# rezashkv/unlearn-ft

Hardware: AMD Instinct MI355X
Metric: bilevel train-step images/sec @512^2 pruned-SD2.1 (higher is better)
Workload: dtype bf16; 1 GPU; BASELINE configs[1] model+batch (MAC-budget-0.55 SD-2.1 student [ratio 0.556, 223.7 GMAC/img] + dense teacher [402.1 GMAC/img], B=8/GPU, 64x64 latents = 512^2 px, losses 1.0 ddpm(min-SNR 5) + 2.0 distill + 0.1 block) under the bilevel cadence of configs[2] (upper concept-suppression step every 10th iteration, second AdamW); global_batch=8, parallelism=dp1, student_params=483766084, weights=random-init, attention_precision=activation dtype, dist_backend=none, rccl_ranks=0, dp_mode=allreduce, teacher_prefetch=True

## Files before the change

include/pdmk.h:

```cpp
#ifndef PDMK_H
#define PDMK_H
#include <stdint.h>
#ifdef __cplusplus
extern "C" {
#endif

#define PDMK_F32 0
#define PDMK_BF16 1

typedef void* pdmk_stream;

int pdmk_version(void);

#define PDMK_A_ROWK 0
#define PDMK_A_CONV 1
#define PDMK_A_COLK 2
#define PDMK_B_ROWK 0
#define PDMK_B_COLK 1
#define PDMK_B_COLK_CONV 2

typedef struct pdmk_gemm_args {
    const void* A;
    const void* B;
    void* C;
    const float* bias;
    const float* rowvec;
    const void* R;
    float* colsum_out;
    int32_t M, N, K;
    int32_t lda, ldb, ldc, ldr;
    int32_t rows_per_b;
    int32_t a_mode, b_mode;
    int32_t conv_b, conv_hi, conv_wi, conv_ci, conv_ho, conv_wo, conv_mode, conv_ld;
    int32_t dtype;
    int32_t out_f32;
    int32_t accumulate;
    int32_t splitk;
    float alpha;
    int32_t ldrv;
    int32_t epilogue;
    int32_t ldc2;
    void* C2;
    int64_t* colstat;
    int32_t cs_ld;
    int32_t cs_col0;
    const float* ln_gamma;
    const float* ln_beta;
    float* ln_stats;
    void* ln_out;
    int32_t ld_ln_out;
    float ln_eps;
} pdmk_gemm_args;
int pdmk_gemm_ln_supported(const pdmk_gemm_args* args);

#define PDMK_EPI_NONE 0
#define PDMK_EPI_GEGLU 1
#define PDMK_EPI_GEGLU_BWD 2

int pdmk_gemm(const pdmk_gemm_args* args, pdmk_stream stream);
int pdmk_conv_up2_supported(int B, int H, int W, int Ci, int Co, int dtype);
int pdmk_groupnorm_apply_colstat(const void* x, void* y, const float* gamma, const float* beta, float* stats, const int64_t* colstat,
                                 int cs_ld, int cs_col0, int B, int HW, int C, int ldx, int ldy, int G, int gs, float eps,
                                 int silu, int dtype, pdmk_stream stream);
int pdmk_up2_pack_weights(const float* w3, void* wp, void* wpt, int Co, int Ci, int dtype, pdmk_stream stream);
int pdmk_up2_combine_wgrad(const float* dwp, float* dw3, int Co, int Ci, pdmk_stream stream);
#define PDMK_COLSTAT_SCALE 1073741824.0
#define PDMK_GEMM_GROUP_MAX 8
int pdmk_gemm_group(const pdmk_gemm_args* args, int n, pdmk_stream stream, int32_t* grouped_out);
int pdmk_gemm_plan(const pdmk_gemm_args* args, pdmk_stream stream, int32_t* splitk_out);
int pdmk_gemm_last_candidate(void);
int pdmk_gemm_candidate_name(int a_mode, int b_mode, int id, char* buf, int n);
int pdmk_splitk_finish(const float* ws, void* C, const float* bias, const float* rowvec, const void* R, int64_t M,
                       int N, int ldc, int ldr, int rows_per_b, int ldrv , int nslab ,
                       int accumulate, int dtype, pdmk_stream stream);
int pdmk_splitk_finish_colstat(const float* ws, void* C, const float* bias, const float* rowvec, const void* R, int64_t M,
                               int N, int ldc, int ldr, int rows_per_b, int ldrv, int nslab, int accumulate, int64_t* colstat,
                               int cs_ld, int cs_col0, int dtype, pdmk_stream stream);
#define PDMK_SLAB_GROUP_MAX 32
typedef struct pdmk_slab_item {
    const float* ws;
    float* dst;
    int64_t n;
    int32_t nslab, pad_;
} pdmk_slab_item;
int pdmk_splitk_finish_group(const pdmk_slab_item* items, int n_items, pdmk_stream stream);
int64_t pdmk_gemm_splitk_workspace_bytes(int64_t M, int N, int splitk);

int pdmk_plan_export(const char* path);
int pdmk_plan_import(const char* path);
int pdmk_plan_size(void);
int pdmk_plan_clear(void);
int pdmk_debug_scratch_violations(void);

int pdmk_groupnorm_fwd(const void* x, void* y, const float* gamma, const float* beta, float* stats, double* ws,
                       int B, int HW, int C, int ldx, int ldy, int G, int gs, float eps, int silu, int dtype,
                       pdmk_stream stream);
int pdmk_groupnorm_bwd(const void* x, const void* dy, void* dx, const float* gamma, const float* beta,
                       const float* stats, float* dgamma, float* dbeta, double* ws, float* part_ws,
                       int64_t part_ws_elems, int B, int HW, int C, int ldx, int lddy, int lddx, int G, int gs,
                       int silu, int accumulate_dx, const void* add, int ldadd, int dtype, pdmk_stream stream);
#define PDMK_PARTIAL_GROUP_MAX 32
typedef struct pdmk_partial_item {
    const float* part;
    float* out0;
    float* out1;
    int32_t nblk, n;
} pdmk_partial_item;
int pdmk_groupnorm_bwd_partial_dims(int B, int HW, int C, int G, int gs, int dtype, int32_t* nblk, int32_t* n);
int pdmk_layernorm_bwd_partial_dims(int M, int C, int32_t* nblk, int32_t* n);
int pdmk_reduce_partials_group(const pdmk_partial_item* items, int n_items, pdmk_stream stream);
int64_t pdmk_groupnorm_workspace_bytes(int B, int G);
int64_t pdmk_groupnorm_bwd_part_workspace_bytes(int G, int gs);

int pdmk_layernorm_fwd(const void* x, void* y, const float* gamma, const float* beta, float* stats, int M, int C,
                       int ldx, int ldy, float eps, int dtype, pdmk_stream stream);
int pdmk_layernorm_bwd(const void* x, const void* dy, void* dx, const float* gamma, const float* stats,
                       float* dgamma, float* dbeta, float* part_ws, int64_t part_ws_elems ,
                       int M, int C, int ldx, int lddy, int lddx, int accumulate_dx, const void* add, int ldadd, int dtype,
                       pdmk_stream stream);
int64_t pdmk_layernorm_bwd_part_workspace_bytes(int M, int C);

int pdmk_attn_fwd(const void* q, const void* k, const void* v, void* o, float* lse, int B, int H, int Nq, int Nk,
                  int64_t q_bs, int q_ld, int64_t k_bs, int k_ld, int64_t v_bs, int v_ld, int64_t o_bs, int o_ld,
                  float scale, int dtype, pdmk_stream stream);
int pdmk_attn_bwd(const void* q, const void* k, const void* v, const void* o, const void* d_o, const float* lse,
                  float* delta, void* dq, void* dk, void* dv, int B, int H, int Nq, int Nk, int64_t q_bs, int q_ld,
                  int64_t k_bs, int k_ld, int64_t v_bs, int v_ld, int64_t o_bs, int o_ld, int64_t dq_bs, int dq_ld,
                  int64_t dk_bs, int dk_ld, int64_t dv_bs, int dv_ld, float scale, float* ws, int64_t ws_elems,
                  int dtype, pdmk_stream stream);
int64_t pdmk_attn_bwd_workspace_bytes(int B, int H, int Nq, int Nk);

int pdmk_geglu_fwd(const void* x, void* y, int M, int F, int ldx, int ldy, int layout, int dtype, pdmk_stream stream);
int pdmk_geglu_bwd(const void* x, const void* dy, void* dx, int M, int F, int ldx, int lddy, int lddx, int layout,
                   int dtype, pdmk_stream stream);
int pdmk_silu_fwd(const void* x, void* y, int64_t n, int dtype, pdmk_stream stream);
int pdmk_quantize_e4m3(const void* x, void* y, int64_t n, int dtype, pdmk_stream stream);
int pdmk_silu_bwd(const void* x, const void* dy, void* dx, int64_t n, int dtype, pdmk_stream stream);
int pdmk_copy2d(const void* src, void* dst, int64_t rows, int cols, int lds, int ldd, int accumulate, int dtype,
                pdmk_stream stream);
int pdmk_cast_permute(const float* src, void* dst, int n0, int n1, int n2, int mode, int dtype, pdmk_stream stream);
int pdmk_colsum(const void* x, float* out, int64_t rows, int N, int ld, int accumulate, int nbatch, int ldo , int dtype, pdmk_stream stream);
int pdmk_pool2x2_sum(const void* src, void* dst, int B, int H, int W, int C, int dtype, pdmk_stream stream);
int pdmk_timestep_embed(const int64_t* t, const float* freqs, void* out, int B, int dim, int dtype,
                        pdmk_stream stream);
int pdmk_add_noise_velocity(const float* x0, const float* noise, const int64_t* t, const float* sqrt_acp,
                            const float* sqrt_1macp, void* noisy_nhwc, float* target_nhwc, int B, int C, int HW,
                            int cpad, int dtype, pdmk_stream stream);
int pdmk_nchw_to_nhwc(const float* src, void* dst, int B, int C, int HW, int cpad, int dtype, pdmk_stream stream);
int pdmk_nhwc_to_nchw(const void* src, float* dst, int B, int C, int HW, int ld, int dtype, pdmk_stream stream);

int pdmk_mse_fwd(const void* a, int a_dtype, const void* b, int b_dtype, const float* w, double* out, int slot,
                 int B, int64_t rows_per_b, int cols, int lda, int ldb, double scale, pdmk_stream stream);
int pdmk_mse_bwd(const void* a, int a_dtype, const void* b, int b_dtype, const float* w, void* da, int B,
                 int64_t rows_per_b, int cols, int lda, int ldb, int ldda, float gscale, int accumulate,
                 pdmk_stream stream);
int pdmk_mse_fwd_bwd(const void* a, int a_dtype, const void* b, int b_dtype, const float* w, double* out, int slot,
                     void* da, int B, int64_t rows_per_b, int cols, int lda, int ldb, int ldda, double scale,
                     float gscale, int accumulate, pdmk_stream stream);
int pdmk_zero(void* p, int64_t nbytes, pdmk_stream stream);
int pdmk_axpby(const void* x, void* y, float alpha, float beta, int64_t n, int dtype, pdmk_stream stream);

int pdmk_adamw(float* p, float* g, float* m, float* v, int64_t n, const float* lr, float beta1, float beta2,
               float eps, float weight_decay, const float* bias_corr , float grad_scale,
               int zero_grad, void* w_bf16 , pdmk_stream stream);
int pdmk_transpose_tiles(const void* src, void* dst, const int32_t* table, int ntiles, int dtype, pdmk_stream stream);
int pdmk_skinny_gemm(const void* x, int x_dtype, const void* w, void* y, const float* bias, int M, int N, int K,
                     int ldx, int ldw, int ldy, int dtype, int out_f32, int accumulate, pdmk_stream stream);
int pdmk_skinny_wgrad(const void* dy, int dy_dtype, const void* x, float* dw, float* dbias, int M, int N, int K,
                      int lddy, int ldx, int lddw, int dtype, pdmk_stream stream);
int pdmk_sumsq(const float* x, int64_t n, double* out, int slot, pdmk_stream stream);

int pdmk_softmax_rows(const float* s, void* p, int64_t rows, int cols, int64_t lds, int64_t ldp, int dtype,
                      pdmk_stream stream);
int pdmk_latent_sample(const void* moments, int ld, const float* eps, float* latents, int B, int C, int HW, float scale,
                       int dtype, pdmk_stream stream);

int pdmk_embed_tokens(const int64_t* ids, const void* tok, const void* pos, void* out, int64_t ntok, int T, int D,
                      int vocab, int ldt, int ldp, int ldo, int dtype, pdmk_stream stream);
int pdmk_attn_fwd_causal(const void* q, const void* k, const void* v, void* o, float* lse, int B, int H, int N,
                         int64_t q_bs, int q_ld, int64_t k_bs, int k_ld, int64_t v_bs, int v_ld, int64_t o_bs, int o_ld,
                         float scale, int dtype, pdmk_stream stream);
int pdmk_gelu_fwd(const void* x, void* y, int64_t n, int dtype, pdmk_stream stream);

typedef struct {
    int64_t offset;
    int64_t h, w;
    int64_t rh, rw;
    int64_t top, left;
    int64_t flip;
} pdmk_image_desc;
int pdmk_image_prep(const uint8_t* src, int64_t src_bytes, const pdmk_image_desc* desc, const pdmk_image_desc* desc_dev,
                    int B, int R, float* out, pdmk_stream stream);
int pdmk_image_prep_ex(const uint8_t* src, int64_t src_bytes, const pdmk_image_desc* desc, const pdmk_image_desc* desc_dev,
                       int B, int R, int filter, const float* mean, const float* stdv, float* out, pdmk_stream stream);

int pdmk_patch_im2col(const float* x, void* out, int B, int S, int p, int ldo, int dtype, pdmk_stream stream);
int pdmk_vit_tokens(const void* patches, int ldp, const void* cls, const void* pos, int ldpos, void* out, int ldo, int B,
                    int G2, int E, int dtype, pdmk_stream stream);
int pdmk_quick_gelu_fwd(const void* x, void* y, int64_t n, int dtype, pdmk_stream stream);
int pdmk_gather_rows(const void* x, int ldx, const int64_t* ids, int T, void* out, int ldo, int B, int D, int dtype,
                     pdmk_stream stream);
int pdmk_clip_score_head(const float* a, int lda, const float* b, int ldb, float* an, float* bn, double* acc, int B, int D,
                         pdmk_stream stream);

typedef struct {
    int64_t t;
    int32_t mode;
    int32_t nterms;
    int32_t wslot;
    int32_t rslot[3];
    float coef[4];
    float v_x, v_v;
    float eps_scale, x_scale;
    int32_t vpred;
    int32_t pad_;
} pdmk_plms_row;

int pdmk_plms_step(const void* pred, int ld, float g_u, float g_t, int cfg, float* sample, float* cur, float* ets,
                   const pdmk_plms_row* table, int nsteps, int32_t* state, int64_t* t_out, void* x_next, int cpad,
                   int B, int C, int HW, int dtype, pdmk_stream stream);

int pdmk_image_to_u8(const float* src, uint8_t* dst, int B, int C, int HW, pdmk_stream stream);
// ... 30 lines not shown
```

unlearn-ft_amd/csrc/gemm.hip:

```cpp
#include <cstdio>
#include <cstdlib>
#include <cstring>
#include <map>
#include <mutex>
#include <vector>

#include "common.h"
#include <algorithm>

namespace {

#define PDMK_GEMM_NBUF 2
#ifndef PDMK_GEMM_PF2
#define PDMK_GEMM_PF2 0
#endif
constexpr int BM = 128, BN = 128;
template <typename T, int KCHUNKS, int NW> struct TileCfg {
    static constexpr int NTHREADS = 64 * NW;
    static constexpr int IM = 8 / NW * 2;
    static constexpr int TPR = NTHREADS / 128;
    static constexpr int NLD = KCHUNKS / TPR;
    static constexpr int ROW_BYTES = KCHUNKS == 8 ? 144 : 96;
    static constexpr int OPERAND_BYTES = 128 * ROW_BYTES;
    static constexpr int CH = Mma<T>::CH;
// ... 276 lines not shown
                for (int h = 0; h < 2; ++h) {
                    const int n = n0 + h * 64 + lane;
                    if (n < g.N) {
                        float v = stage[lrow * SROW + h * 64 + lane];
                        if (first) {
                            if (g.bias) v += g.bias[n];
                            if (g.rowvec) v += g.rowvec[(long)(m / g.rows_per_b) * (g.ldrv ? g.ldrv : g.N) + n];
                            if (Rp) v += to_f32(Rp[(long)m * g.ldr + n]);
                        }
                        unsafeAtomicAdd(Cf + (long)m * g.ldc + n, v);
                    }
                }
            }
        } else {
            constexpr int TPS = NTHREADS / 64, SEG = 128 / TPS;
            const int lrow = tid / TPS, seg = (tid % TPS) * SEG;
            const int m = m0 + pass * 64 + lrow;
            if (m < g.M) {
                const float* rv = g.rowvec ? g.rowvec + (long)(m / g.rows_per_b) * (g.ldrv ? g.ldrv : g.N) : nullptr;
#pragma unroll
                for (int c8 = 0; c8 < SEG / 8; ++c8) {
                    const int n = n0 + seg + c8 * 8;
                    if (n >= g.N) break;
                    float v[8];
                    const f32x4 lo = *reinterpret_cast<const f32x4*>(stage + lrow * SROW + seg + c8 * 8);
                    const f32x4 hi = *reinterpret_cast<const f32x4*>(stage + lrow * SROW + seg + c8 * 8 + 4);
#pragma unroll
                    for (int r = 0; r < 4; ++r) { v[r] = lo[r]; v[4 + r] = hi[r]; }
                    const long off = (long)m * g.ldc + n;
                    if (vec8) {
                        if (g.bias) {
                            const float4 b0 = *reinterpret_cast<const float4*>(g.bias + n), b1 = *reinterpret_cast<const float4*>(g.bias + n + 4);
                            v[0] += b0.x; v[1] += b0.y; v[2] += b0.z; v[3] += b0.w; v[4] += b1.x; v[5] += b1.y; v[6] += b1.z; v[7] += b1.w;
                        }
                        if (rv) {
                            const float4 b0 = *reinterpret_cast<const float4*>(rv + n), b1 = *reinterpret_cast<const float4*>(rv + n + 4);
                            v[0] += b0.x; v[1] += b0.y; v[2] += b0.z; v[3] += b0.w; v[4] += b1.x; v[5] += b1.y; v[6] += b1.z; v[7] += b1.w;
                        }
                        if (Rp) {
                            if (sizeof(T) == 2) {
                                const bf16x8 rr = *reinterpret_cast<const bf16x8*>(Rp + (long)m * g.ldr + n);
#pragma unroll
                                for (int r = 0; r < 8; ++r) v[r] += (float)rr[r];
                            } else {
                                const float* rp = reinterpret_cast<const float*>(Rp) + (long)m * g.ldr + n;
                                const float4 b0 = *reinterpret_cast<const float4*>(rp), b1 = *reinterpret_cast<const float4*>(rp + 4);
                                v[0] += b0.x; v[1] += b0.y; v[2] += b0.z; v[3] += b0.w; v[4] += b1.x; v[5] += b1.y; v[6] += b1.z; v[7] += b1.w;
                            }
                        }
                        if (f32out) {
                            float4 o0 = make_float4(v[0], v[1], v[2], v[3]), o1 = make_float4(v[4], v[5], v[6], v[7]);
                            if (acc1) {
                                const float4 c0 = *reinterpret_cast<const float4*>(Cf + off), c1 = *reinterpret_cast<const float4*>(Cf + off + 4);
                                o0.x += c0.x; o0.y += c0.y; o0.z += c0.z; o0.w += c0.w; o1.x += c1.x; o1.y += c1.y; o1.z += c1.z; o1.w += c1.w;
                            }
                            *reinterpret_cast<float4*>(Cf + off) = o0;
                            *reinterpret_cast<float4*>(Cf + off + 4) = o1;
                        } else {
                            if (acc1) {
                                const bf16x8 c = *reinterpret_cast<const bf16x8*>(Ct + off);
#pragma unroll
                                for (int r = 0; r < 8; ++r) v[r] += (float)c[r];
                            }
                            bf16x8 o;
#pragma unroll
                            for (int r = 0; r < 8; ++r) o[r] = (bf16)v[r];
                            st_stream(reinterpret_cast<bf16x8*>(Ct + off), o);
                        }
                    } else {
                        const int nv = min(8, g.N - n);
                        for (int r = 0; r < nv; ++r) {
                            float x = v[r];
                            if (g.bias) x += g.bias[n + r];
                            if (rv) x += rv[n + r];
                            if (Rp) x += to_f32(Rp[(long)m * g.ldr + n + r]);
                            if (f32out) Cf[off + r] = x + (acc1 ? Cf[off + r] : 0.f);
                            else Ct[off + r] = from_f32<T>(x + (acc1 ? to_f32(Ct[off + r]) : 0.f));
                        }
                    }
                }
            }
        }
    }
}

inline int ilog2_exact(int v) {
    if (v <= 0 || (v & (v - 1))) return -1;
    int l = 0;
    while ((1 << l) < v) ++l;
    return l;
}

template <typename T> int launch(const pdmk_gemm_args& g, hipStream_t st) {
    const int mt = (g.M + BM - 1) / BM, nt = (g.N + BN - 1) / BN;
    dim3 grid(mt * nt, g.splitk > 1 ? g.splitk : 1);
    int lg_wo = -1, lg_howo = -1;
    if (g.b_mode == PDMK_B_COLK_CONV) {
        lg_wo = ilog2_exact(g.conv_wo);
        lg_howo = ilog2_exact(g.conv_ho * g.conv_wo);
        if (lg_wo < 0 || lg_howo < 0) lg_wo = lg_howo = -1;
    }
    const long esz = sizeof(T);
    const long conv_bytes = (((long)g.conv_b * g.conv_hi * g.conv_wi - 1) * g.conv_ld + g.conv_ci) * esz;
    const long a_bytes = g.a_mode == PDMK_A_ROWK ? ((long)(g.M - 1) * g.lda + g.K) * esz
                       : g.a_mode == PDMK_A_CONV ? conv_bytes : ((long)(g.K - 1) * g.lda + g.M) * esz;
    const long b_bytes = g.b_mode == PDMK_B_ROWK ? ((long)(g.N - 1) * g.ldb + g.K) * esz
                       : g.b_mode == PDMK_B_COLK ? ((long)(g.K - 1) * g.ldb + g.N) * esz : conv_bytes;
    if (a_bytes >= (1L << 31) || b_bytes >= (1L << 31)) return -1;
    const bool many = (long)grid.x * grid.y > 512;
    const bool deep4 = false;
#define PDMK_GO(AM, BMD, CM)                                                                                        \
    do {                                                                                                            \
        if (deep4)                                                                                                  \
            hipLaunchKernelGGL((igemm_kernel<T, AM, BMD, CM, 4, 4>), grid, dim3(256), 0, st, g, lg_wo, lg_howo,     \
                               (unsigned)a_bytes, (unsigned)b_bytes);                                               \
        else if (many)                                                                                              \
            hipLaunchKernelGGL((igemm_kernel<T, AM, BMD, CM, 4, 8>), grid, dim3(512), 0, st, g, lg_wo, lg_howo,     \
                               (unsigned)a_bytes, (unsigned)b_bytes);                                               \
        else                                                                                                        \
            hipLaunchKernelGGL((igemm_kernel<T, AM, BMD, CM, 8, 8>), grid, dim3(512), 0, st, g, lg_wo, lg_howo,     \
                               (unsigned)a_bytes, (unsigned)b_bytes);                                               \
    } while (0)
    if (g.a_mode == PDMK_A_ROWK && g.b_mode == PDMK_B_ROWK) PDMK_GO(PDMK_A_ROWK, PDMK_B_ROWK, 0);
    else if (g.a_mode == PDMK_A_CONV && g.b_mode == PDMK_B_ROWK) {
        switch (g.conv_mode) {
            case 0: PDMK_GO(PDMK_A_CONV, PDMK_B_ROWK, 0); break;
            case 1: PDMK_GO(PDMK_A_CONV, PDMK_B_ROWK, 1); break;
            case 2: PDMK_GO(PDMK_A_CONV, PDMK_B_ROWK, 2); break;
            case 3: PDMK_GO(PDMK_A_CONV, PDMK_B_ROWK, 3); break;
            default: PDMK_GO(PDMK_A_CONV, PDMK_B_ROWK, 4); break;
        }
    } else if (g.a_mode == PDMK_A_COLK && g.b_mode == PDMK_B_COLK) PDMK_GO(PDMK_A_COLK, PDMK_B_COLK, 0);
    else if (g.a_mode == PDMK_A_COLK && g.b_mode == PDMK_B_COLK_CONV) {
        switch (g.conv_mode) {
            case 0: PDMK_GO(PDMK_A_COLK, PDMK_B_COLK_CONV, 0); break;
            case 1: PDMK_GO(PDMK_A_COLK, PDMK_B_COLK_CONV, 1); break;
            case 2: PDMK_GO(PDMK_A_COLK, PDMK_B_COLK_CONV, 2); break;
            default: return -2;
        }
    } else return -2;
#undef PDMK_GO
    PDMK_CHECK_LAUNCH();
    return 0;
}

}

int pdmk_gemm_dma_launch(const pdmk_gemm_args& g, hipStream_t st, long a_bytes, long b_bytes);
int pdmk_gemm_ring_launch(const pdmk_gemm_args& g, hipStream_t st, long a_bytes, long b_bytes, int id);
int pdmk_gemm_ring_num_configs();
int pdmk_gemm_ring_pick(const pdmk_gemm_args& g);
int pdmk_wgrad_ring_launch(const pdmk_gemm_args& g, hipStream_t st, long a_bytes, long b_bytes, int id);
int pdmk_wgrad_ring_num_configs();

static int env_int(const char* name, int def, int* cache) {
    static int dynamic = -1;
    if (dynamic < 0) dynamic = getenv("PDMK_ENV_DYNAMIC") ? 1 : 0;
    if (*cache == INT32_MIN || dynamic) {
        const char* e = getenv(name);
        *cache = e ? atoi(e) : def;
    }
    return *cache;
}
static int dma_mode() { static int c = INT32_MIN; return env_int("PDMK_GEMM_DMA", 1, &c); }
static int ring_mode() { static int c = INT32_MIN; return env_int("PDMK_GEMM_RING", 1, &c); }
static int tune_mode() { static int c = INT32_MIN; return env_int("PDMK_GEMM_TUNE", 1, &c); }
static int forced_cfg() { static int c = INT32_MIN; return env_int("PDMK_RING_CFG", -1, &c); }
static int forced_wcfg() { static int c = INT32_MIN; return env_int("PDMK_WGRAD_CFG", -1, &c); }

namespace {

struct PlanKey {
    int v[10];
    bool operator<(const PlanKey& o) const { return memcmp(v, o.v, sizeof v) < 0; }
};
std::mutex g_plan_mu;
std::map<PlanKey, int> g_plan_cfg;
std::map<PlanKey, int> g_plan_sk;
thread_local int g_last_candidate = -1;
bool g_plan_file_loaded = false;

void plan_file_load() {
    if (g_plan_file_loaded) return;
    g_plan_file_loaded = true;
    const char* path = getenv("PDMK_PLAN_CACHE");
    if (!path) return;
    FILE* f = fopen(path, "r");
    if (!f) return;
    int ver = 0;
    if (fscanf(f, " pdmk-plan %d", &ver) != 1 || ver != pdmk_version()) {
        fclose(f);
        return;
    }
    char kind;
    PlanKey k;
    int val;
    while (fscanf(f, " %c %d %d %d %d %d %d %d %d %d %d %d", &kind, &k.v[0], &k.v[1], &k.v[2], &k.v[3], &k.v[4], &k.v[5],
                  &k.v[6], &k.v[7], &k.v[8], &k.v[9], &val) == 12) {
        if (kind == 'c') g_plan_cfg[k] = val;
        else if (kind == 's') g_plan_sk[k] = val;
    }
    fclose(f);
}
void plan_file_append(char kind, const PlanKey& k, int val) {
    const char* path = getenv("PDMK_PLAN_CACHE");
    if (!path) return;
    FILE* probe = fopen(path, "r");
    int ver = 0;
    const bool fresh = !probe || fscanf(probe, " pdmk-plan %d", &ver) != 1 || ver != pdmk_version();
    if (probe) fclose(probe);
    FILE* f = fopen(path, fresh ? "w" : "a");
    if (!f) return;
    if (fresh) fprintf(f, "pdmk-plan %d\n", pdmk_version());
    fprintf(f, "%c %d %d %d %d %d %d %d %d %d %d %d\n", kind, k.v[0], k.v[1], k.v[2], k.v[3], k.v[4], k.v[5], k.v[6], k.v[7],
            k.v[8], k.v[9], val);
    fclose(f);
}
void* g_scratch = nullptr;
size_t g_scratch_bytes = 0;

PlanKey make_key(const pdmk_gemm_args& g, int sk) {
    PlanKey k;
    const bool cv = g.a_mode == PDMK_A_CONV || g.b_mode == PDMK_B_COLK_CONV;
    const int slabw = (g.a_mode == PDMK_A_COLK && g.accumulate == 2) ? 1000 : 0;
    const int v[10] = {g.M, g.N, g.K, g.a_mode, g.b_mode, (cv ? g.conv_mode : 100 * g.epilogue) + slabw, cv ? g.conv_hi : 0,
                       cv ? g.conv_wi : 0, cv ? g.conv_ci : 0, sk};
    memcpy(k.v, v, sizeof v);
    return k;
}

bool ring_eligible(const pdmk_gemm_args& g) {
    return g.dtype == PDMK_BF16 && g.b_mode == PDMK_B_ROWK && g.a_mode != PDMK_A_COLK;
}

bool wgrad_eligible(const pdmk_gemm_args& g) {
    return g.dtype == PDMK_BF16 && g.a_mode == PDMK_A_COLK && g.b_mode != PDMK_B_ROWK && g.out_f32 &&
           (g.b_mode == PDMK_B_COLK || g.conv_mode <= 2 || (g.conv_mode >= 5 && g.conv_mode <= 8));
}

bool operand_bytes(const pdmk_gemm_args& g, long* ab, long* bb) {
    const long in_px = (long)g.conv_b * g.conv_hi * g.conv_wi * ((g.a_mode == PDMK_A_CONV && g.conv_mode >= 9) ? 4 : 1);
    const long conv_bytes = ((in_px - 1) * g.conv_ld + g.conv_ci) * 2;
    const long krows = (g.a_mode == PDMK_A_COLK && g.b_mode == PDMK_B_COLK_CONV && g.conv_mode >= 5) ? 4L * g.K : (long)g.K;
    *ab = g.a_mode == PDMK_A_ROWK ? ((long)(g.M - 1) * g.lda + g.K) * 2
        : g.a_mode == PDMK_A_CONV ? conv_bytes : ((krows - 1) * g.lda + g.M) * 2;
    *bb = g.b_mode == PDMK_B_ROWK ? ((long)(g.N - 1) * g.ldb + g.K) * 2
        : g.b_mode == PDMK_B_COLK ? ((long)(g.K - 1) * g.ldb + g.N) * 2 : conv_bytes;
    return *ab < (1L << 31) && *bb < (1L << 31);
}

int launch_legacy(const pdmk_gemm_args& g, hipStream_t st) {
    if (g.colstat) return -2;
    if ((g.a_mode == PDMK_A_CONV || g.b_mode == PDMK_B_COLK_CONV) && g.conv_mode >= 5) return -2;
    const long nblocks = (long)((g.M + 127) / 128) * ((g.N + 127) / 128) * (g.splitk > 1 ? g.splitk : 1);
    long ab, bb;
    if (dma_mode() && (nblocks >= 384 || dma_mode() == 2) && ring_eligible(g) && (g.K % 32) == 0 && operand_bytes(g, &ab, &bb)) {
        const int rc = pdmk_gemm_dma_launch(g, st, ab, bb);
        if (rc <= 0) return rc;
    }
    return g.dtype == PDMK_BF16 ? launch<bf16>(g, st) : launch<float>(g, st);
}

int launch_candidate(const pdmk_gemm_args& g, hipStream_t st, int id) {
    if (id <= 0) return launch_legacy(g, st);
    long ab, bb;
    if (!operand_bytes(g, &ab, &bb)) return 1;
    if (g.a_mode == PDMK_A_COLK) return pdmk_wgrad_ring_launch(g, st, ab, bb, id - 1);
    return pdmk_gemm_ring_launch(g, st, ab, bb, id - 1);
}

static int debug_scratch();
long out_rows(const pdmk_gemm_args& g) {
    const bool phase_fwd = g.a_mode == PDMK_A_CONV && g.conv_mode >= 5 && g.conv_mode <= 8;
    if (phase_fwd && debug_scratch() == 2 && 3L * g.M * g.N * 4 + 4096 <= (1L << 20)) return (long)g.M;
    return phase_fwd ? 4L * g.M : (long)g.M;
}

bool can_tune(hipStream_t st) {
    if (!tune_mode() || !ring_mode()) return false;
    hipStreamCaptureStatus cs = hipStreamCaptureStatusNone;
    if (hipStreamIsCapturing(st, &cs) != hipSuccess) { (void)hipGetLastError(); return false; }
    return cs == hipStreamCaptureStatusNone;
}

constexpr size_t kCanaryBytes = 1 << 20;
size_t g_scratch_req = 0;
int g_scratch_violations = 0;
static int debug_scratch() { static int c = INT32_MIN; return env_int("PDMK_DEBUG_SCRATCH", 0, &c); }
static_assert(kCanaryBytes == (1 << 20), "out_rows() sizes its deliberate overrun against the band");

bool ensure_scratch(size_t bytes) {
    if (debug_scratch()) {
        if (g_scratch) (void)hipFree(g_scratch);
        g_scratch = nullptr;
        g_scratch_bytes = 0;
        bytes = (bytes + 255) & ~(size_t)255;
        if (hipMalloc(&g_scratch, bytes + kCanaryBytes) != hipSuccess) { (void)hipGetLastError(); return false; }
        if (hipMemset(reinterpret_cast<char*>(g_scratch) + bytes, 0xA5, kCanaryBytes) != hipSuccess) { (void)hipGetLastError(); return false; }
        (void)hipDeviceSynchronize();
        g_scratch_bytes = bytes + kCanaryBytes;
        g_scratch_req = bytes;
        return true;
    }
    if (bytes <= g_scratch_bytes) return true;
    if (g_scratch) (void)hipFree(g_scratch);
    g_scratch = nullptr;
// ... 102 lines not shown
    if (s > 64) s = 64;
    return s < 1 ? 1 : s;
}

int heuristic_sk(const pdmk_gemm_args& g) {
    if (g.N & 3) return 1;
    const bool conv0 = g.a_mode == PDMK_A_CONV && g.conv_mode == 0;
    const int bm = conv0 ? (g.M >= 8192 ? 256 : 128) : (g.M >= 8192 ? 128 : 64);
    const int bn = conv0 ? 160 : 128;
    const long tiles = (long)((g.M + bm - 1) / bm) * ((g.N + bn - 1) / bn);
    const int nk = (g.K + 63) / 64;
    if (tiles >= 160 || nk < 30) return 1;
    long s = (256 + tiles - 1) / tiles;
    if (s > nk / 8) s = nk / 8;
    if (conv0 && s > (g.conv_ci + 63) / 64) s = (g.conv_ci + 63) / 64;
    return s < 1 ? 1 : (s > 16 ? 16 : (int)s);
}

}

static int validate_args(const pdmk_gemm_args& g) {
    if (!g.A || !g.B || !g.C) return -1;
    if (g.M <= 0 || g.N <= 0 || g.K <= 0) return -1;
    const int ch = g.dtype == PDMK_BF16 ? 8 : 4;
    const int g4 = 4 * ch;
    if (g.dtype != PDMK_BF16 && g.dtype != PDMK_F32) return -2;
    if (g.a_mode != PDMK_A_COLK && (g.K % g4)) return -1;
    if (((uintptr_t)g.A | (uintptr_t)g.B) & 15) return -1;
    if (g.a_mode == PDMK_A_ROWK && (g.lda % ch)) return -1;
    if (g.a_mode == PDMK_A_COLK && ((g.lda % ch) || (g.M % g4))) return -1;
    if (g.b_mode == PDMK_B_ROWK && (g.ldb % ch)) return -1;
    if (g.b_mode == PDMK_B_COLK && ((g.ldb % ch) || (g.N % g4))) return -1;
    if (g.a_mode == PDMK_A_CONV || g.b_mode == PDMK_B_COLK_CONV) {
        if (g.conv_ci <= 0 || (g.conv_ci % g4) || (g.conv_ld % ch) || g.conv_mode < 0 || g.conv_mode > 13) return -1;
        if (g.conv_mode >= 5) {
            if (g.dtype != PDMK_BF16 || g.conv_ho != g.conv_hi || g.conv_wo != g.conv_wi) return -2;
            if (g.b_mode == PDMK_B_COLK_CONV && g.conv_mode > 8) return -1;
        }
        if (g.conv_mode == 4 && (g.b_mode == PDMK_B_COLK_CONV || (g.conv_hi & 1) || (g.conv_wi & 1))) return -1;
        if (g.conv_b <= 0 || g.conv_hi <= 0 || g.conv_wi <= 0 || g.conv_ho <= 0 || g.conv_wo <= 0) return -1;
        const long px = (long)g.conv_b * g.conv_ho * g.conv_wo;
        if (px >= (1L << 30) || (long)g.conv_b * g.conv_hi * g.conv_wi >= (1L << 30)) return -1;
        const int ntaps = g.conv_mode == 13 ? 16 : (g.conv_mode >= 5 ? 4 : 9);
        if (g.a_mode == PDMK_A_CONV && (g.M != px || g.K != ntaps * g.conv_ci)) return -1;
        if (g.b_mode == PDMK_B_COLK_CONV && (g.K != px || g.N != ntaps * g.conv_ci)) return -1;
        if (g.conv_mode >= 5 && (long)g.conv_b * g.conv_hi * g.conv_wi * 4 >= (1L << 30)) return -1;
        const bool half = g.conv_mode == 1 || g.conv_mode == 4, twice = g.conv_mode == 2 || g.conv_mode == 3;
        const int eh = half ? (g.conv_hi + 1) / 2 : (twice ? 2 * g.conv_hi : g.conv_hi);
        const int ew = half ? (g.conv_wi + 1) / 2 : (twice ? 2 * g.conv_wi : g.conv_wi);
        if (g.conv_ho != eh || g.conv_wo != ew) return -1;
    }
    if (g.splitk > 1 && !(g.out_f32 || g.dtype == PDMK_F32)) return -1;
    if (g.accumulate == 2 && (g.splitk <= 1 || !(g.out_f32 || g.dtype == PDMK_F32) || g.bias || g.rowvec || g.R)) return -1;
    if (g.accumulate < 0 || g.accumulate > 2) return -1;
    if (g.rowvec && g.rows_per_b <= 0) return -1;
    if (g.epilogue != PDMK_EPI_NONE) {
        if (g.epilogue != PDMK_EPI_GEGLU && g.epilogue != PDMK_EPI_GEGLU_BWD) return -2;
        if (g.dtype != PDMK_BF16 || g.a_mode != PDMK_A_ROWK || g.b_mode != PDMK_B_ROWK || g.out_f32) return -2;
        if (g.epilogue == PDMK_EPI_GEGLU) {
            if ((g.N % 16) || (g.ldc % 8) || (g.C2 && (g.ldc2 % 8)) || g.splitk > 1 || g.accumulate || g.R || g.rowvec ||
                g.alpha != 1.0f || (g.K % 8))
                return -1;
        } else {
            if ((g.N % 8) || (g.ldc % 8) || !g.C2 || (g.ldc2 % 8) || g.splitk > 1 || g.accumulate || g.R || g.rowvec || g.bias ||
                g.alpha != 1.0f || (g.K % 8) || (((uintptr_t)g.C2 | (uintptr_t)g.C) & 15))
                return -1;
        }
        if (!ring_mode()) return -2;
    }
    if (g.colstat) {
        if (g.dtype != PDMK_BF16 || g.a_mode == PDMK_A_COLK || g.b_mode != PDMK_B_ROWK || g.out_f32 || g.epilogue) return -2;
        if (g.rows_per_b <= 0 || (g.rows_per_b % 64) || (g.M % 64) || (g.N % 8) || (g.ldc % 8) || (g.R && (g.ldr % 8)) ||
            g.splitk > 1 || g.accumulate == 2 || g.cs_col0 < 0 || g.cs_ld < g.cs_col0 + g.N || (g.K % 8))
            return -1;
        if (g.a_mode == PDMK_A_CONV && g.conv_mode >= 9) return -1;
        if (!ring_mode()) return -2;
    }
    return 0;
}

int pdmk_gemm_rowblock_launch(const pdmk_gemm_args& g, hipStream_t st, long a_bytes, long b_bytes, int id, bool dry);
int pdmk_gemm_rowblock_num_configs();
static int ln_candidate(const pdmk_gemm_args& g, long* ab, long* bb) {
    if (g.dtype != PDMK_BF16 || g.a_mode != PDMK_A_ROWK || g.b_mode != PDMK_B_ROWK || g.splitk > 1 || g.colstat || g.out_f32 ||
        !ring_mode() || !operand_bytes(g, ab, bb))
        return -1;
    for (int id = 0; id < pdmk_gemm_rowblock_num_configs(); ++id)
        if (pdmk_gemm_rowblock_launch(g, nullptr, *ab, *bb, id, true) == 0) return id;
    return -1;
}
extern "C" int pdmk_gemm_ln_supported(const pdmk_gemm_args* a) {
    if (!a || !a->ln_gamma || validate_args(*a)) return 0;
    long ab, bb;
    return ln_candidate(*a, &ab, &bb) >= 0 ? 1 : 0;
}

extern "C" int pdmk_gemm(const pdmk_gemm_args* a, pdmk_stream stream) {
    if (!a) return -1;
    const pdmk_gemm_args& g = *a;
    if (const int vrc = validate_args(g)) return vrc;
    hipStream_t st = reinterpret_cast<hipStream_t>(stream);
    g_last_candidate = 0;
    if (g.ln_gamma) {
        long ab, bb;
        const int id = ln_candidate(g, &ab, &bb);
        if (id < 0) return -2;
        const int rc = pdmk_gemm_rowblock_launch(g, st, ab, bb, id, false);
        g_last_candidate = 1 + pdmk_gemm_ring_num_configs() - pdmk_gemm_rowblock_num_configs() + id;
        return rc == 1 ? -2 : rc;
    }
    if (!(ring_eligible(g) && (g.K % 8) == 0) && !wgrad_eligible(g)) return launch_legacy(g, st);
    if ((g.a_mode == PDMK_A_COLK ? forced_wcfg() >= 0 : forced_cfg() >= 0) && !(g.epilogue && forced_cfg() == 0)) {
        const int rc = launch_candidate(g, st, g.a_mode == PDMK_A_COLK ? forced_wcfg() : forced_cfg());
        g_last_candidate = rc == 1 ? 0 : (g.a_mode == PDMK_A_COLK ? forced_wcfg() : forced_cfg());
        if (g.epilogue && rc == 1) return -2;
        const bool phase = (g.a_mode == PDMK_A_CONV || g.b_mode == PDMK_B_COLK_CONV) && g.conv_mode >= 5;
        if (!((phase || g.colstat) && rc == 1)) return rc == 1 ? launch_legacy(g, st) : rc;
    }
    const int sk = g.splitk > 1 ? g.splitk : 1;
    int id;
    {
        std::lock_guard<std::mutex> lk(g_plan_mu);
        plan_file_load();
        const PlanKey key = make_key(g, sk);
        auto it = g_plan_cfg.find(key);
        if (it != g_plan_cfg.end()) id = it->second;
        else if (can_tune(st)) {
            float t;
            id = tune_cfg(g, st, sk, &t);
            if (id < 0) id = heuristic_cfg(g);
            g_plan_cfg[key] = id;
            plan_file_append('c', key, id);
        } else id = heuristic_cfg(g);
    }
    if ((g.epilogue || g.colstat) && id <= 0) id = 1 + pdmk_gemm_ring_pick(g);
    int rc = launch_candidate(g, st, id);
    if (g.colstat && rc == 1) {
        id = 1 + pdmk_gemm_ring_pick(g);
        rc = launch_candidate(g, st, id);
    }
    if (g.epilogue && rc == 1) return -2;
    g_last_candidate = rc == 1 ? 0 : id;
    return rc == 1 ? launch_legacy(g, st) : rc;
}

int pdmk_gemm_ring_group_launch(const pdmk_gemm_args* gs, int n, hipStream_t st, const long* a_bytes, const long* b_bytes, int id);
int pdmk_wgrad_ring_group_launch(const pdmk_gemm_args* gs, int n, hipStream_t st, const long* a_bytes, const long* b_bytes, int id);
static int group_mode() { static int c = INT32_MIN; return env_int("PDMK_GEMM_GROUP", 1, &c); }
static int forced_group() { static int c = INT32_MIN; return env_int("PDMK_GROUP_CFG", -1, &c); }

namespace {

std::map<std::vector<int>, int> g_group_plan;

int member_plan(const pdmk_gemm_args& g, hipStream_t st) {
    const int sk = g.splitk > 1 ? g.splitk : 1;
    std::lock_guard<std::mutex> lk(g_plan_mu);
    plan_file_load();
    const PlanKey key = make_key(g, sk);
    auto it = g_plan_cfg.find(key);
    if (it != g_plan_cfg.end()) return it->second;
    if (!can_tune(st)) return heuristic_cfg(g);
    float t;
    int id = tune_cfg(g, st, sk, &t);
    if (id < 0) id = heuristic_cfg(g);
    g_plan_cfg[key] = id;
    plan_file_append('c', key, id);
    return id;
}

int group_launch(const pdmk_gemm_args* a, int n, hipStream_t st, int id) {
    long ab[PDMK_GEMM_GROUP_MAX], bb[PDMK_GEMM_GROUP_MAX];
    for (int i = 0; i < n; ++i)
        if (!operand_bytes(a[i], &ab[i], &bb[i])) return 1;
    if (id <= 0) return 1;
    if (a[0].a_mode == PDMK_A_COLK) return pdmk_wgrad_ring_group_launch(a, n, st, ab, bb, id - 1);
    return pdmk_gemm_ring_group_launch(a, n, st, ab, bb, id - 1);
}

template <typename F> float time_us(F fn, hipStream_t st, hipEvent_t e0, hipEvent_t e1, int reps = 3) {
    if (fn() != 0) { (void)hipGetLastError(); return 1e30f; }
    float best = 1e30f;
    for (int round = 0; round < 2; ++round) {
        (void)hipEventRecord(e0, st);
        for (int r = 0; r < reps; ++r)
            if (fn() != 0) { (void)hipGetLastError(); return 1e30f; }
        (void)hipEventRecord(e1, st);
        if (hipEventSynchronize(e1) != hipSuccess) { (void)hipGetLastError(); return 1e30f; }
        float ms = 0.f;
        (void)hipEventElapsedTime(&ms, e0, e1);
        if (ms < best) best = ms;
    }
    return best * 1000.f / reps;
}

int tune_group(const pdmk_gemm_args* a, int n, const int* ids, hipStream_t st) {
    pdmk_gemm_args t[PDMK_GEMM_GROUP_MAX];
    size_t off[PDMK_GEMM_GROUP_MAX + 1];
    off[0] = 0;
    for (int i = 0; i < n; ++i) {
        const size_t out = (size_t)out_rows(a[i]) * (size_t)a[i].N * 4;
        const size_t slabs = (a[i].accumulate == 2 && a[i].splitk > 1) ? (size_t)a[i].splitk : 1;
        off[i + 1] = off[i] + ((out * slabs + (size_t)a[i].M * 4 + 1023) & ~(size_t)1023);
    }
    {
        std::lock_guard<std::mutex> lk(g_plan_mu);
        if (!ensure_scratch(off[n] + 256)) return -1;
    }
    (void)hipDeviceSynchronize();
    for (int i = 0; i < n; ++i) {
        t[i] = a[i];
        char* base = reinterpret_cast<char*>(g_scratch) + off[i];
        t[i].C = base;
        t[i].ldc = a[i].N;
        t[i].colstat = nullptr;
        if (t[i].epilogue == PDMK_EPI_GEGLU_BWD) t[i].ldc = 2 * a[i].N;
        else t[i].C2 = nullptr;
        if (t[i].accumulate == 1) t[i].accumulate = 0;
        if (t[i].epilogue == PDMK_EPI_GEGLU) t[i].ldc = a[i].N / 2;
        if (t[i].colsum_out)
            t[i].colsum_out = reinterpret_cast<float*>(base + (off[i + 1] - off[i]) - (((size_t)a[i].M * 4 + 15) & ~(size_t)15));
    }
    hipEvent_t e0, e1;
    if (hipEventCreate(&e0) != hipSuccess || hipEventCreate(&e1) != hipSuccess) { (void)hipGetLastError(); return -1; }
    const float t_sep = time_us([&]() -> int {
        for (int i = 0; i < n; ++i) {
            int rc = launch_candidate(t[i], st, ids[i]);
            if (rc == 1) rc = launch_legacy(t[i], st);
            if (rc) return rc;
        }
        return 0;
    }, st, e0, e1);
    int best = -1;
    float bt = t_sep * 0.98f;
    int cands[PDMK_GEMM_GROUP_MAX + 12], nc = 0;
    for (int i = 0; i < n; ++i) cands[nc++] = ids[i];
    cands[nc++] = heuristic_cfg(a[0]);
    if (a[0].a_mode == PDMK_A_CONV)
        for (int h = 0; h < 4; ++h) cands[nc++] = 1 + 12 + h;
    if (a[0].a_mode == PDMK_A_COLK && a[0].b_mode == PDMK_B_COLK)
        for (int w = 0; w < 5; ++w) cands[nc++] = 1 + w;
    for (int i = 0; i < nc; ++i) {
        bool seen = cands[i] <= 0;
        for (int j = 0; j < i; ++j) seen = seen || cands[j] == cands[i];
        if (seen) continue;
        const float tg = time_us([&]() -> int { return group_launch(t, n, st, cands[i]); }, st, e0, e1);
        if (tg < bt) { bt = tg; best = cands[i]; }
    }
    (void)hipEventDestroy(e0);
    (void)hipEventDestroy(e1);
    if (getenv("PDMK_TUNE_LOG")) {
        fprintf(stderr, "[pdmk group] n=%d", n);
        for (int i = 0; i < n; ++i) fprintf(stderr, " (%d,%d,%d|a%d sk%d id%d)", a[i].M, a[i].N, a[i].K, a[i].a_mode, a[i].splitk, ids[i]);
        fprintf(stderr, " separate %.1f us -> %s %d (%.1f us)\n", t_sep, best > 0 ? "grouped cand" : "separate", best, best > 0 ? bt : t_sep);
    }
    {
        std::lock_guard<std::mutex> lk(g_plan_mu);
        if (!scratch_check()) return -1;
    }
    return best;
}

}

extern "C" int pdmk_gemm_group(const pdmk_gemm_args* a, int n, pdmk_stream stream, int32_t* grouped_out) {
    if (grouped_out) *grouped_out = 0;
    if (!a || n < 1 || n > PDMK_GEMM_GROUP_MAX) return -1;
    bool any_ln = false;
    for (int i = 0; i < n; ++i) {
        if (const int vrc = validate_args(a[i])) return vrc;
        any_ln = any_ln || a[i].ln_gamma;
    }
    hipStream_t st = reinterpret_cast<hipStream_t>(stream);
    auto separate = [&]() -> int {
        for (int i = 0; i < n; ++i)
            if (const int rc = pdmk_gemm(&a[i], stream)) return rc;
        return 0;
    };
    if (n > 1 && forced_group() >= 1 && !any_ln) {
        const int rc = group_launch(a, n, st, forced_group());
        if (rc == 0) {
            g_last_candidate = forced_group();
            if (grouped_out) *grouped_out = n;
            return 0;
        }
        return rc == 1 ? separate() : rc;
    }
    if (n == 1 || any_ln || !group_mode() || !ring_mode() || forced_cfg() >= 0 || forced_wcfg() >= 0) return separate();
    bool fw = true, wg = true;
    for (int i = 0; i < n; ++i) {
        fw = fw && ring_eligible(a[i]) && (a[i].K % 8) == 0 && (a[i].a_mode == a[0].a_mode);
        wg = wg && wgrad_eligible(a[i]) && (a[i].b_mode == a[0].b_mode);
    }
    if (!fw && !wg) return separate();
    int ids[PDMK_GEMM_GROUP_MAX];
    std::vector<int> key;
    for (int i = 0; i < n; ++i) {
        ids[i] = member_plan(a[i], st);
        if ((a[i].epilogue || a[i].colstat) && ids[i] <= 0) ids[i] = 1 + pdmk_gemm_ring_pick(a[i]);
        const PlanKey k = make_key(a[i], a[i].splitk > 1 ? a[i].splitk : 1);
        key.insert(key.end(), k.v, k.v + 10);
        key.push_back(a[i].accumulate);
    }
    int id = -2;
    {
        std::lock_guard<std::mutex> lk(g_plan_mu);
        auto it = g_group_plan.find(key);
        if (it != g_group_plan.end()) id = it->second;
    }
    if (id == -2) {
        if (can_tune(st)) {
            id = tune_group(a, n, ids, st);
            std::lock_guard<std::mutex> lk(g_plan_mu);
            g_group_plan[key] = id;
        } else {
            id = ids[0];
            for (int i = 1; i < n; ++i)
                if (ids[i] != ids[0]) id = -1;
        }
    }
    if (id > 0) {
        const int rc = group_launch(a, n, st, id);
        if (rc == 0) {
            g_last_candidate = id;
            if (grouped_out) *grouped_out = n;
            return 0;
        }
        if (rc != 1) return rc;
    }
    return separate();
}

extern "C" int pdmk_gemm_last_candidate(void) { return g_last_candidate; }
int pdmk_gemm_ring_name(int id, int conv, char* buf, int n);
int pdmk_wgrad_ring_name(int id, int conv, char* buf, int n);
extern "C" int pdmk_gemm_candidate_name(int a_mode, int b_mode, int id, char* buf, int n) {
    if (!buf || n <= 0) return -1;
    if (id <= 0) {
        snprintf(buf, n, "igemm_kernel / pdmk_dma::igemm_dma_kernel (K-step-32)");
        return 0;
    }
    if (a_mode == PDMK_A_COLK) return pdmk_wgrad_ring_name(id - 1, b_mode == PDMK_B_COLK_CONV, buf, n);
    return pdmk_gemm_ring_name(id - 1, a_mode == PDMK_A_CONV, buf, n);
}

extern "C" int pdmk_gemm_plan(const pdmk_gemm_args* a, pdmk_stream stream, int32_t* splitk_out) {
    if (!a || !splitk_out) return -1;
    const pdmk_gemm_args& g = *a;
    hipStream_t st = reinterpret_cast<hipStream_t>(stream);
    *splitk_out = 1;
    if (g.M <= 0 || g.N <= 0 || g.K <= 0) return -1;
    if ((g.N & 3) || g.epilogue) return 0;
    const bool wg = wgrad_eligible(g);
    if (g.a_mode == PDMK_A_COLK && !wg) {
        *splitk_out = heuristic_wgrad_sk(g);
        return 0;
    }
    if (!wg && (!ring_eligible(g) || (g.K % 8) || forced_cfg() >= 0)) {
        *splitk_out = heuristic_sk(g);
        return 0;
    }
    std::lock_guard<std::mutex> lk(g_plan_mu);
    plan_file_load();
    const PlanKey key0 = make_key(g, 0);
    auto it = g_plan_sk.find(key0);
    if (it != g_plan_sk.end()) { *splitk_out = it->second; return 0; }
    if (!can_tune(st) || !a->A || !a->B) { *splitk_out = wg ? heuristic_wgrad_sk(g) : heuristic_sk(g); return 0; }
    const int tiles = ((g.M + 127) / 128) * ((g.N + 127) / 128);
    const int nk = (g.K + 63) / 64;
    const int cands[12] = {1, 2, 3, 4, 6, 8, 12, 16, 24, 32, 48, 64};
    int best_sk = 1;
    float bt = 1e30f;
    for (int c = 0; c < 12; ++c) {
        const int sk = cands[c];
        if (wg) {
            if (sk > 1 && (nk / sk < 4 || (long)tiles * sk > 1280)) continue;
            if ((long)tiles * sk * 4 < 128 && sk < 64 && nk / (2 * sk) >= 4) continue;
        } else if (sk > 16 || (sk > 1 && (tiles > 200 || nk < 10 || nk / sk < 3 || (long)tiles * sk > 768))) continue;
        float t = 1e30f;
        const int id = tune_cfg(g, st, sk, &t);
        if (id < 0) continue;
        g_plan_cfg[make_key(g, sk)] = id;
        plan_file_append('c', make_key(g, sk), id);
        static const float margin = getenv("PDMK_SPLIT_MARGIN") ? 1.0f - 0.01f * (float)atof(getenv("PDMK_SPLIT_MARGIN")) : 0.97f;
        if (t < bt * (sk > 1 ? margin : 1.0f)) { bt = t; best_sk = sk; }
    }
    g_plan_sk[key0] = best_sk;
    plan_file_append('s', key0, best_sk);
    *splitk_out = best_sk;
    return 0;
}

extern "C" int pdmk_plan_size(void) {
    std::lock_guard<std::mutex> lk(g_plan_mu);
    return (int)(g_plan_cfg.size() + g_plan_sk.size());
}
extern "C" int pdmk_plan_export(const char* path) {
    if (!path) return -1;
    std::lock_guard<std::mutex> lk(g_plan_mu);
    FILE* f = fopen(path, "w");
    if (!f) return -1;
    fprintf(f, "pdmk-plan %d\n", pdmk_version());
    for (int pass = 0; pass < 2; ++pass)
        for (const auto& kv : (pass ? g_plan_sk : g_plan_cfg)) {
            const PlanKey& k = kv.first;
            fprintf(f, "%c %d %d %d %d %d %d %d %d %d %d %d\n", pass ? 's' : 'c', k.v[0], k.v[1], k.v[2], k.v[3], k.v[4], k.v[5],
                    k.v[6], k.v[7], k.v[8], k.v[9], kv.second);
        }
    return fclose(f) == 0 ? 0 : -1;
}
extern "C" int pdmk_plan_import(const char* path) {
    if (!path) return -1;
    std::lock_guard<std::mutex> lk(g_plan_mu);
    FILE* f = fopen(path, "r");
    if (!f) return -1;
    int ver = 0;
    if (fscanf(f, " pdmk-plan %d", &ver) != 1 || ver != pdmk_version()) {
        fclose(f);
        return -2;
    }
    char kind;
    PlanKey k;
    int val, n = 0;
    while (fscanf(f, " %c %d %d %d %d %d %d %d %d %d %d %d", &kind, &k.v[0], &k.v[1], &k.v[2], &k.v[3], &k.v[4], &k.v[5],
                  &k.v[6], &k.v[7], &k.v[8], &k.v[9], &val) == 12) {
        if (kind == 'c') g_plan_cfg[k] = val;
        else if (kind == 's') g_plan_sk[k] = val;
        ++n;
    }
    fclose(f);
    return n;
}
extern "C" int pdmk_plan_clear(void) {
    std::lock_guard<std::mutex> lk(g_plan_mu);
    g_plan_cfg.clear();
    g_plan_sk.clear();
    g_group_plan.clear();
    if (g_scratch) (void)hipFree(g_scratch);
    g_scratch = nullptr;
    g_scratch_bytes = 0;
    return 0;
}

extern "C" int pdmk_debug_scratch_violations(void) {
    std::lock_guard<std::mutex> lk(g_plan_mu);
    return g_scratch_violations;
}

extern "C" int pdmk_version(void) { return 121; }
```

unlearn-ft_amd/csrc/gemm_ring.hip:

```cpp
#include "common.h"

#include <stdio.h>
#include <stdlib.h>

#ifndef PDMK_WGRAD_XCD
#define PDMK_WGRAD_XCD 1
#endif
#ifndef PDMK_HALO_PAIRS
#define PDMK_HALO_PAIRS 1
#endif
#ifndef PDMK_RING_SPLIT_ISSUE
#define PDMK_RING_SPLIT_ISSUE 0
#endif
#ifndef PDMK_HALO_SPLIT_ISSUE
#define PDMK_HALO_SPLIT_ISSUE 1
#endif

#ifndef PDMK_PRIO
#define PDMK_PRIO 0
#endif

namespace pdmk_ring {

constexpr int BK = 64, NT = 512;
constexpr unsigned OOB = 0x80000000u;
typedef __attribute__((address_space(3))) void lds_void;

struct ConvGeom {
    int hi, wi, ci, ho, wo, ld, mode;
};

struct LC {
    unsigned bx, by, gx, gy;
};
__device__ __forceinline__ LC lc_plain() { return LC{blockIdx.x, blockIdx.y, gridDim.x, gridDim.y}; }
__device__ __forceinline__ LC lc_split_xcd() {
    const unsigned gx = gridDim.x, gy = gridDim.y;
    if (gy == 1) return LC{blockIdx.x, 0u, gx, 1u};
    const unsigned t = (unsigned)xcd_remap((int)(blockIdx.y * gx + blockIdx.x), (int)(gx * gy));
    const unsigned z = t / gx;
    return LC{t - z * gx, z, gx, gy};
}
__device__ __forceinline__ bool lc_group(const pdmk_gemm_group_dev& gg, int& pi, LC& lc) {
    const unsigned b = blockIdx.x;
    pi = 0;
#pragma unroll
    for (int i = 1; i < PDMK_GEMM_GROUP_MAX; ++i)
        if (i < gg.n && b >= (unsigned)gg.start[i]) pi = i;
    const unsigned local = b - (unsigned)gg.start[pi];
    const unsigned gx = (unsigned)gg.gx[pi], gy = (unsigned)gg.gy[pi];
    if (local >= gx * gy) return false;
    const unsigned t = gy > 1 ? (unsigned)xcd_remap((int)local, (int)(gx * gy)) : local;
    const unsigned z = t / gx;
    lc = LC{t - z * gx, z, gx, gy};
    return true;
}

__device__ __forceinline__ int conv_src_pixel(const ConvGeom& g, int b, int oy, int ox, int tap) {
    if (g.mode >= 5) {
        const int ph = g.mode - 5, vy = oy + (tap >> 1) - 1 + (ph >> 1), vx = ox + (tap & 1) - 1 + (ph & 1);
        const bool ok = (unsigned)vy < (unsigned)g.hi && (unsigned)vx < (unsigned)g.wi && tap < 4;
        return ok ? (b * g.hi + vy) * g.wi + vx : -1;
    }
    const int ky = (tap * 11) >> 5;
    const int kx = tap - 3 * ky;
    const bool s2 = g.mode == 1 || g.mode == 4, up = g.mode == 2 || g.mode == 3;
    const int pad = g.mode == 4 ? 0 : 1;
    const int vy = (s2 ? 2 * oy : oy) + ky - pad, vx = (s2 ? 2 * ox : ox) + kx - pad;
    const int hv = up ? 2 * g.hi : g.hi, wv = up ? 2 * g.wi : g.wi;
    bool ok = (unsigned)vy < (unsigned)hv && (unsigned)vx < (unsigned)wv && tap < 9;
    if (g.mode == 3) ok = ok && (((vy | vx) & 1) == 0);
    const int iy = up ? (vy >> 1) : vy, ix = up ? (vx >> 1) : vx;
    return ok ? (b * g.hi + iy) * g.wi + ix : -1;
}

__device__ __forceinline__ void wait_vmcnt_dyn(int n) { pdmk_wait_vmcnt(n); }
__device__ __forceinline__ void prio_static(int wave) {
    if (PDMK_PRIO == 1 && wave >= 4) __builtin_amdgcn_s_setprio(1);
}
#define PDMK_PRIO_UP() do { if (PDMK_PRIO == 2) __builtin_amdgcn_s_setprio(1); } while (0)
#define PDMK_PRIO_DOWN() do { if (PDMK_PRIO == 2) __builtin_amdgcn_s_setprio(0); } while (0)

template <int BM, int NJ, int LDS_BYTES, bool TILE2D = false, bool OUTMAP = false>
__device__ __forceinline__ void ring_epilogue(const pdmk_gemm_args& g, const LC wgc, f32x4 (&acc)[BM / 64][NJ], unsigned char* smem,
                                              int m0, int n0, int tw = 0, int img_w = 0) {
    auto row_of = [&](int l) { return TILE2D ? m0 + (l / tw) * img_w + (l % tw) : m0 + l; };
    auto out_row = [&](int m) -> long {
        if (!OUTMAP) return (long)m;
        const int hw = g.conv_hi * g.conv_wi, b = m / hw, rem = m - b * hw, y = rem / g.conv_wi, x = rem - y * g.conv_wi;
        const int ph = g.conv_mode - 5;
        return ((long)(b * 2 * g.conv_hi + 2 * y + (ph >> 1)) * (2 * g.conv_wi) + 2 * x + (ph & 1));
    };
    constexpr int BN = 32 * NJ, IM = BM / 64;
    const int tid = threadIdx.x, lane = tid & 63, wave = __builtin_amdgcn_readfirstlane(tid >> 6);
    const int wm = wave >> 1, wn = wave & 1;
    const bool first = wgc.by == 0;
    const bool slab = g.accumulate == 2;
    const bool atomic = wgc.gy > 1 && !slab;
    const bool acc1 = g.accumulate == 1;
    const bool f32out = g.out_f32 != 0;
    const bool vec8 = ((g.N & 7) == 0) && ((g.ldc & 7) == 0) && (g.R == nullptr || (g.ldr & 7) == 0);
    constexpr int SROW = BN + 4;
    constexpr int C8 = BN / 8;
    constexpr int ITEMS = (64 * C8 + NT - 1) / NT;
    constexpr int RS = NT / C8, CS_STRIDE = RS * C8, ITEMS_CS = (64 + RS - 1) / RS;
    constexpr bool CS_OK = RS * 2 * BN * 4 <= LDS_BYTES;
    static_assert(ITEMS_CS >= ITEMS && (CS_OK || NJ < 2), "statistics epilogue of the forward tile shapes");
    float* stage = reinterpret_cast<float*>(smem);
    static_assert(64 * SROW * 4 <= LDS_BYTES, "staging image must fit the ring");
    float* Cf = reinterpret_cast<float*>(g.C) + (slab ? (long)wgc.by * g.M * g.ldc : 0L);
    bf16* Ct = reinterpret_cast<bf16*>(g.C);
    const bf16* Rp = reinterpret_cast<const bf16*>(g.R);
    float cs1[8] = {0.f, 0.f, 0.f, 0.f, 0.f, 0.f, 0.f, 0.f}, cs2[8] = {0.f, 0.f, 0.f, 0.f, 0.f, 0.f, 0.f, 0.f};
#pragma unroll
    for (int pass = 0; pass < BM / 64; ++pass) {
        __syncthreads();
        if ((wm * 16 * IM) / 64 == pass) {
            const int lrb = (wm * 16 * IM) % 64;
#pragma unroll
            for (int i = 0; i < IM; ++i)
#pragma unroll
                for (int j = 0; j < NJ; ++j) {
                    f32x4 v = acc[i][j];
#pragma unroll
                    for (int r = 0; r < 4; ++r) v[r] *= g.alpha;
                    *reinterpret_cast<f32x4*>(stage + (lrb + i * 16 + (lane & 15)) * SROW + wn * (16 * NJ) + j * 16 + (lane >> 4) * 4) = v;
                }
        }
        if (atomic) {
            __syncthreads();
            for (int rr = 0; rr < 8; ++rr) {
                const int lr2 = wave * 8 + rr, m = row_of(pass * 64 + lr2);
                if (m >= g.M) break;
#pragma unroll
                for (int h = 0; h < (BN + 63) / 64; ++h) {
                    const int cl = h * 64 + lane, n = n0 + cl;
                    if (cl < BN && n < g.N) {
                        float v = stage[lr2 * SROW + cl];
                        if (first) {
                            if (g.bias) v += g.bias[n];
                            if (g.rowvec) v += g.rowvec[(long)(m / g.rows_per_b) * (g.ldrv ? g.ldrv : g.N) + n];
                            if (Rp) v += (float)Rp[(long)m * g.ldr + n];
                        }
                        unsafeAtomicAdd(Cf + (long)m * g.ldc + n, v);
                    }
                }
            }
        } else if (vec8 && g.epilogue == PDMK_EPI_GEGLU) {
            constexpr int C16 = BN / 16;
            constexpr int ITEMS2 = (64 * C16 + NT - 1) / NT;
            bf16* C2 = reinterpret_cast<bf16*>(g.C2);
            __syncthreads();
#pragma unroll
            for (int it = 0; it < ITEMS2; ++it) {
                const int item = tid + it * NT;
                const int lr2 = item / C16, p = item - lr2 * C16;
// ... 656 lines not shown
    const int per = (nk_total + wgc.gy - 1) / wgc.gy;
    const int kt0 = wgc.by * per;
    const int kt1 = min(nk_total, kt0 + per);
    if (kt0 >= kt1 && g.accumulate != 2) return;

    const auto rsrcA = __builtin_amdgcn_make_buffer_rsrc(const_cast<void*>(g.A), (short)0, (int)a_bytes, 0x00020000);
    const auto rsrcB = __builtin_amdgcn_make_buffer_rsrc(const_cast<void*>(g.B), (short)0, (int)b_bytes, 0x00020000);
    const ConvGeom cg{g.conv_hi, g.conv_wi, g.conv_ci, g.conv_ho, g.conv_wo, g.conv_ld, g.conv_mode};

    auto lane_row = [&](int rbytes) { return rbytes == 256 ? (lane >> 4) : (lane >> 3); };
    auto lane_lc = [&](int rbytes) {
        if (rbytes == 256) return (lane & 15) ^ (((lane >> 4) | (((wave >> 1) & 1) << 2)) << 1);
        return (lane & 7) ^ (((((lane >> 3) >> 1) & 1) | ((wave & 1) << 1)) << 1);
    };
    const int a_row = lane_row(RA), b_rowl = lane_row(RB);
    const int acol = m0 + lane_lc(RA) * 8, bcol = n0 + lane_lc(RB) * 8;
    const bool a_ok = acol < g.M, b_ok = bcol < g.N;
    int b_tap = 0, b_ci = 0;
    if (CONV) {
        b_tap = bcol / cg.ci;
        b_ci = bcol - b_tap * cg.ci;
    }

    auto issue = [&](int kt, int slot) {
        unsigned char* sa = smem + slot * SLOT;
#pragma unroll
        for (int i = 0; i < PA; ++i) {
            const int piece = i * 8 + wave;
            const int kr = kt * BK + piece * (1024 / RA) + a_row;
            unsigned krs = (unsigned)kr;
            if (CONV && cg.mode >= 5 && kr < g.K) {
                const int hw = cg.ho * cg.wo, b = kr / hw, rem = kr - b * hw, oy = rem / cg.wo, ox = rem - oy * cg.wo;
                const int ph = cg.mode - 5;
                krs = (unsigned)((b * 2 * cg.ho + 2 * oy + (ph >> 1)) * (2 * cg.wo) + 2 * ox + (ph & 1));
            }
            const unsigned va = (kr < g.K && a_ok) ? (krs * (unsigned)g.lda + (unsigned)acol) * 2u : OOB;
            __builtin_amdgcn_raw_ptr_buffer_load_lds(rsrcA, (lds_void*)(sa + piece * 1024), 16, (int)va, 0, 0, 0);
        }
#pragma unroll
        for (int i = 0; i < PB; ++i) {
            const int piece = i * 8 + wave;
            const int kr = kt * BK + piece * (1024 / RB) + b_rowl;
            const bool kok = kr < g.K;
            unsigned vb = OOB;
            if (CONV) {
                if (kok && b_ok) {
                    int b, oy, ox;
                    if (lg_wo >= 0) {
                        b = kr >> lg_howo;
                        const int rem = kr & ((1 << lg_howo) - 1);
                        oy = rem >> lg_wo;
                        ox = rem & ((1 << lg_wo) - 1);
                    } else {
                        const int hw = cg.ho * cg.wo;
                        b = kr / hw;
                        const int rem = kr - b * hw;
                        oy = rem / cg.wo;
                        ox = rem - oy * cg.wo;
                    }
                    const int px = conv_src_pixel(cg, b, oy, ox, b_tap);
                    if (px >= 0) vb = ((unsigned)px * (unsigned)cg.ld + (unsigned)b_ci) * 2u;
                }
            } else if (kok && b_ok) {
                vb = ((unsigned)kr * (unsigned)g.ldb + (unsigned)bcol) * 2u;
            }
            __builtin_amdgcn_raw_ptr_buffer_load_lds(rsrcB, (lds_void*)(sa + A_BYTES + piece * 1024), 16, (int)vb, 0, 0, 0);
        }
    };

    f32x4 acc[IM][NJ], acs[IM];
#pragma unroll
    for (int i = 0; i < IM; ++i) {
        acs[i] = f32x4{0.f, 0.f, 0.f, 0.f};
#pragma unroll
        for (int j = 0; j < NJ; ++j) acc[i][j] = f32x4{0.f, 0.f, 0.f, 0.f};
    }
    const bool do_colsum = g.colsum_out != nullptr && n0 == 0 && wn == 0;
    bf16x8 ones;
#pragma unroll
    for (int e = 0; e < 8; ++e) ones[e] = (bf16)1.0f;

    const int tg = lane >> 4, tq = (lane & 15) >> 2, tp = lane & 3;
    const int f256 = (tq | ((tg & 1) << 2)) << 1, f128 = (((tq >> 1) & 1) | ((tg & 1) << 1)) << 1;
    typedef __attribute__((address_space(3))) s16x4 lds_s16x4;
    auto tr_frag = [&](const unsigned char* base, int rbytes, int kk, int col0) -> bf16x8 {
        const unsigned ch = (unsigned)(((col0 >> 3) ^ (rbytes == 256 ? f256 : f128)) | (tp >> 1));
        const unsigned char* a0 = base + (unsigned)(kk + 8 * tg + tq) * (unsigned)rbytes + ch * 16u + (unsigned)(tp & 1) * 8u;
        s16x4 lo = __builtin_amdgcn_ds_read_tr16_b64_v4i16((lds_s16x4*)(a0));
        s16x4 hi = __builtin_amdgcn_ds_read_tr16_b64_v4i16((lds_s16x4*)(a0 + 4 * rbytes));
        s16x8 v = __builtin_shufflevector(lo, hi, 0, 1, 2, 3, 4, 5, 6, 7);
        return __builtin_bit_cast(bf16x8, v);
    };

#pragma unroll
    for (int s = 0; s < STAGES - 1; ++s)
        if (kt0 + s < kt1) issue(kt0 + s, s);

    int slot = 0;
    prio_static(wave);
    for (int kt = kt0; kt < kt1; ++kt) {
        if (STAGES == 2) asm volatile("s_waitcnt vmcnt(0)" ::: "memory");
        else if (kt + STAGES - 1 <= kt1) asm volatile("s_waitcnt vmcnt(%0)" ::"n"((STAGES - 2) * (PA + PB)) : "memory");
        else wait_vmcnt_dyn(min(STAGES - 2, kt1 - 1 - kt) * (PA + PB));
        __builtin_amdgcn_s_barrier();
        if (kt + STAGES - 1 < kt1) issue(kt + STAGES - 1, slot == 0 ? STAGES - 1 : slot - 1);
        const unsigned char* sa = smem + slot * SLOT;
        const unsigned char* sb = sa + A_BYTES;
#pragma unroll
        for (int kk = 0; kk < BK; kk += 32) {
            bf16x8 af[IM], bf[NJ];
#pragma unroll
            for (int i = 0; i < IM; ++i) af[i] = tr_frag(sa, RA, kk, wm * (16 * IM) + i * 16);
#pragma unroll
            for (int j = 0; j < NJ; ++j) bf[j] = tr_frag(sb, RB, kk, wn * (16 * NJ) + j * 16);
            PDMK_PRIO_UP();
#pragma unroll
            for (int i = 0; i < IM; ++i)
#pragma unroll
                for (int j = 0; j < NJ; ++j) acc[i][j] = MM::mma(bf[j], af[i], acc[i][j]);
            PDMK_PRIO_DOWN();
            if (do_colsum) {
#pragma unroll
                for (int i = 0; i < IM; ++i) acs[i] = MM::mma(ones, af[i], acs[i]);
            }
        }
        slot = slot + 1 == STAGES ? 0 : slot + 1;
    }
    if (PDMK_PRIO == 1) __builtin_amdgcn_s_setprio(0);
    if (do_colsum && (lane >> 4) == 0) {
#pragma unroll
        for (int i = 0; i < IM; ++i) {
            const int m = m0 + wm * (16 * IM) + i * 16 + (lane & 15);
            if (m < g.M) unsafeAtomicAdd(g.colsum_out + m, acs[i][0]);
        }
    }
    ring_epilogue<BM, NJ, STAGES * SLOT>(g, wgc, acc, smem, m0, n0);
}

template <bool CONV, int BM, int NJ, int STAGES, int OCC>
__global__ __launch_bounds__(NT, OCC) void wgrad_ring_kernel(pdmk_gemm_args g, int lg_wo, int lg_howo, unsigned a_bytes,
                                                             unsigned b_bytes) {
    __shared__ __attribute__((aligned(1024))) unsigned char smem[wgrad_smem_bytes(BM, NJ, STAGES)];
    wgrad_ring_body<CONV, BM, NJ, STAGES, OCC>(g, lg_wo, lg_howo, a_bytes, b_bytes, PDMK_WGRAD_XCD ? lc_split_xcd() : lc_plain(), smem);
}
template <bool CONV, int BM, int NJ, int STAGES, int OCC>
__global__ __launch_bounds__(NT, OCC) void wgrad_ring_group_kernel(pdmk_gemm_group_dev gg) {
    __shared__ __attribute__((aligned(1024))) unsigned char smem[wgrad_smem_bytes(BM, NJ, STAGES)];
    int pi;
    LC wgc;
    if (!lc_group(gg, pi, wgc)) return;
    wgrad_ring_body<CONV, BM, NJ, STAGES, OCC>(gg.p[pi], gg.aux0[pi], gg.aux1[pi], gg.a_bytes[pi], gg.b_bytes[pi], wgc, smem);
}

struct Config {
    int bm, nj, stages, occ;
};
static const Config kConfigs[] = {
    {256, 4, 3, 2}, {256, 5, 3, 2}, {128, 4, 4, 2}, {128, 5, 4, 2}, {64, 4, 6, 2}, {64, 5, 5, 2},
    {128, 4, 2, 4}, {64, 4, 3, 4},  {64, 5, 2, 4},  {128, 6, 3, 2}, {64, 6, 4, 2},  {128, 5, 2, 4},
    {64, 2, 4, 4},  {128, 2, 3, 4}, {64, 3, 4, 4},
};
constexpr int kNumConfigs = sizeof(kConfigs) / sizeof(kConfigs[0]);
constexpr int kNumBase = 12;

static int halo_tile_w(const pdmk_gemm_args& g, int h, int splitk) {
    const bool phase = g.conv_mode >= 5 && g.conv_mode <= 13;
    if (g.a_mode != PDMK_A_CONV || !(g.conv_mode == 0 || phase) || g.conv_ho != g.conv_hi || g.conv_wo != g.conv_wi) return 0;
    if (phase && (h < 2 || !PDMK_HALO_PAIRS || g.R || (splitk > 1))) return 0;
    if ((g.conv_ci % 8) || g.conv_wi < 4) return 0;
    if (phase ? ((g.ldb % 8) || g.ldb < (g.conv_mode == 13 ? 16 : 4) * g.conv_ci) : g.ldb != 9 * g.conv_ci) return 0;
    if ((splitk > 1 ? splitk : 1) > (g.conv_ci + 63) / 64) return 0;
    const int bm = h < 2 ? 256 : 128, pmax = h < 2 ? 400 : 264;
    const int H = g.conv_hi, W = g.conv_wi, HW = H * W;
    if (HW < bm) return (bm % HW) == 0 && (bm / HW) * (H + 2) * (W + 2) <= pmax ? W : 0;
    if (HW % bm) return 0;
    static const int pref = getenv("PDMK_HALO_TW") ? atoi(getenv("PDMK_HALO_TW")) : 0;
    if (pref > 0 && pref < W && (W % pref) == 0 && (bm % pref) == 0 && (H % (bm / pref)) == 0 &&
        (bm / pref + 2) * (pref + 2) <= pmax)
        return pref;
    if ((bm % W) == 0 && (bm / W + 2) * (W + 2) <= pmax) return W;
    for (int tw = 128; tw >= 8; tw >>= 1) {
        if (tw >= W || (W % tw) || (bm % tw)) continue;
        const int rows = bm / tw;
        if ((H % rows) == 0 && (rows + 2) * (tw + 2) <= pmax) return tw;
    }
    return 0;
}
static bool halo_ok(const pdmk_gemm_args& g, int h, int splitk) { return halo_tile_w(g, h, splitk) > 0; }

static int pick_config(const pdmk_gemm_args& g, int splitk) {
    enum { R256x128, R256x160, R128x128, R128x160, R64x128, R64x160, S128x128, S64x128, S64x160, R128x192, R64x192, S128x160 };
    const bool n160 = (g.N % 160) == 0 || (g.N > 256 && (g.N % 128) != 0);
    if (g.a_mode == PDMK_A_CONV && g.conv_mode >= 5) return kNumBase + (halo_ok(g, n160 ? 2 : 3, splitk) ? (n160 ? 2 : 3) : (n160 ? 3 : 2));
    if (g.a_mode == PDMK_A_CONV && g.conv_mode == 0) {
        const long t256 = (long)((g.M + 255) / 256) * ((g.N + 159) / 160);
        const int h = (g.M >= 8192 && t256 >= 128) ? (n160 ? 0 : 1) : (n160 ? 2 : 3);
        if (halo_ok(g, h, splitk)) return kNumBase + h;
        if (halo_ok(g, h | 2, splitk)) return kNumBase + (h | 2);
    }
    if (g.M >= 8192) return n160 ? S128x160 : S128x128;
    if (g.M >= 4096) return S64x160;
    if (g.M >= 2048 && n160 && g.N >= 1280) return S64x160;
    return S64x128;
}

}

constexpr int kNumHalo = 4;
int pdmk_gemm_rowblock_num_configs();
int pdmk_gemm_rowblock_name(int id, char* buf, int n);
int pdmk_gemm_rowblock_launch(const pdmk_gemm_args& g, hipStream_t st, long a_bytes, long b_bytes, int id, bool dry = false);
static int conv_halo_launch(const pdmk_gemm_args& g, hipStream_t st, long a_bytes, long b_bytes, int id) {
    using namespace pdmk_ring;
    const int tw = halo_tile_w(g, id, g.splitk);
    if (tw <= 0) return 1;
    const int bm = id < 2 ? 256 : 128, nj = (id & 1) ? 4 : 5;
    const int sk = g.splitk > 1 ? g.splitk : 1;
    const int bn = 32 * nj;
    dim3 grid(((g.M + bm - 1) / bm) * ((g.N + bn - 1) / bn), sk);
    if (g.conv_mode >= 5) {
        if (id == 2) hipLaunchKernelGGL((conv_halo_kernel<128, 5, 4, 264, 4>), grid, dim3(NT), 0, st, g, (unsigned)a_bytes, (unsigned)b_bytes, tw);
        else hipLaunchKernelGGL((conv_halo_kernel<128, 4, 5, 264, 4>), grid, dim3(NT), 0, st, g, (unsigned)a_bytes, (unsigned)b_bytes, tw);
        return hipGetLastError() == hipSuccess ? 0 : -1000;
    }
    switch (id) {
        case 0: hipLaunchKernelGGL((conv_halo_kernel<256, 5, 3, 400>), grid, dim3(NT), 0, st, g, (unsigned)a_bytes, (unsigned)b_bytes, tw); break;
        case 1: hipLaunchKernelGGL((conv_halo_kernel<256, 4, 3, 400>), grid, dim3(NT), 0, st, g, (unsigned)a_bytes, (unsigned)b_bytes, tw); break;
        case 2: hipLaunchKernelGGL((conv_halo_kernel<128, 5, 4, 264>), grid, dim3(NT), 0, st, g, (unsigned)a_bytes, (unsigned)b_bytes, tw); break;
        case 3: hipLaunchKernelGGL((conv_halo_kernel<128, 4, 5, 264>), grid, dim3(NT), 0, st, g, (unsigned)a_bytes, (unsigned)b_bytes, tw); break;
        default: return 1;
    }
    return hipGetLastError() == hipSuccess ? 0 : -1000;
}

extern "C" int pdmk_conv_up2_supported(int B, int H, int W, int Ci, int Co, int dtype) {
    if (dtype != PDMK_BF16 || B <= 0 || H <= 0 || W <= 0 || Ci <= 0 || Co <= 0 || (Ci % 32) || (Co % 32)) return 0;
    pdmk_gemm_args g = {};
    g.a_mode = PDMK_A_CONV;
    g.b_mode = PDMK_B_ROWK;
    g.dtype = PDMK_BF16;
    g.conv_b = B;
    g.conv_hi = g.conv_ho = H;
    g.conv_wi = g.conv_wo = W;
    g.M = B * H * W;
    bool ok = true;
    for (int dir = 0; dir < 2; ++dir) {
        g.conv_mode = dir ? 13 : 5;
        g.conv_ci = dir ? Co : Ci;
        g.N = dir ? Ci : Co;
        g.K = (dir ? 16 : 4) * g.conv_ci;
        g.ldb = g.K;
        ok = ok && (pdmk_ring::halo_tile_w(g, 2, 1) > 0 || pdmk_ring::halo_tile_w(g, 3, 1) > 0);
    }
    return ok ? 1 : 0;
}

int pdmk_gemm_ring_num_configs() { return pdmk_ring::kNumConfigs + kNumHalo + pdmk_gemm_rowblock_num_configs(); }
int pdmk_gemm_ring_name(int id, int conv, char* buf, int n) {
    using namespace pdmk_ring;
    if (id >= kNumConfigs + kNumHalo) return pdmk_gemm_rowblock_name(id - (kNumConfigs + kNumHalo), buf, n);
    if (id < 0) return -1;
    if (id >= kNumBase && id < kNumBase + kNumHalo) {
        const int h = id - kNumBase;
        snprintf(buf, n, "pdmk_ring::conv_halo_kernel<%d, %d, %d, %d, 9>", h < 2 ? 256 : 128, (h & 1) ? 4 : 5,
                 h < 2 ? 3 : ((h & 1) ? 5 : 4), h < 2 ? 400 : 264);
        return 0;
    }
    const Config c = kConfigs[id < kNumBase ? id : id - kNumHalo];
    snprintf(buf, n, "pdmk_ring::igemm_ring_kernel<%s, %d, %d, %d, %d>", conv ? "true" : "false", c.bm, c.nj, c.stages, c.occ);
    return 0;
}
int pdmk_gemm_ring_pick(const pdmk_gemm_args& g) { return pdmk_ring::pick_config(g, g.splitk); }

int pdmk_gemm_ring_launch(const pdmk_gemm_args& g, hipStream_t st, long a_bytes, long b_bytes, int id) {
    using namespace pdmk_ring;
    if (g.dtype != PDMK_BF16 || g.b_mode != PDMK_B_ROWK || g.a_mode == PDMK_A_COLK) return 1;
    if ((g.K % 8) || (g.a_mode == PDMK_A_CONV && (g.conv_ci % 8))) return 1;
    if (g.ln_gamma && id < kNumConfigs + kNumHalo) return 1;
    if (id >= kNumBase && id < kNumBase + kNumHalo) return conv_halo_launch(g, st, a_bytes, b_bytes, id - kNumBase);
    if (g.a_mode == PDMK_A_CONV && g.conv_mode >= 5) return 1;
    if (id >= kNumConfigs + kNumHalo) return pdmk_gemm_rowblock_launch(g, st, a_bytes, b_bytes, id - (kNumConfigs + kNumHalo));
    if (id < 0) return 1;
    const int sk = g.splitk > 1 ? g.splitk : 1;
    const Config c = kConfigs[id < kNumBase ? id : id - kNumHalo];
    const int bn = 32 * c.nj;
    dim3 grid(((g.M + c.bm - 1) / c.bm) * ((g.N + bn - 1) / bn), sk);
    const bool conv = g.a_mode == PDMK_A_CONV;
#define PDMK_RING_GO(BMv, NJv, STv, OCv)                                                                              \
    case (BMv * 1000 + NJv * 100 + STv * 10 + OCv):                                                                   \
        if (conv) hipLaunchKernelGGL((igemm_ring_kernel<true, BMv, NJv, STv, OCv>), grid, dim3(NT), 0, st, g,         \
                                     (unsigned)a_bytes, (unsigned)b_bytes);                                           \
        else hipLaunchKernelGGL((igemm_ring_kernel<false, BMv, NJv, STv, OCv>), grid, dim3(NT), 0, st, g,             \
                                (unsigned)a_bytes, (unsigned)b_bytes);                                                \
        break;
    switch (c.bm * 1000 + c.nj * 100 + c.stages * 10 + c.occ) {
        PDMK_RING_GO(256, 4, 3, 2) PDMK_RING_GO(256, 5, 3, 2) PDMK_RING_GO(128, 4, 4, 2) PDMK_RING_GO(128, 5, 4, 2)
        PDMK_RING_GO(64, 4, 6, 2) PDMK_RING_GO(64, 5, 5, 2) PDMK_RING_GO(128, 4, 2, 4) PDMK_RING_GO(64, 4, 3, 4)
        PDMK_RING_GO(64, 5, 2, 4) PDMK_RING_GO(128, 6, 3, 2) PDMK_RING_GO(64, 6, 4, 2) PDMK_RING_GO(128, 5, 2, 4)
        PDMK_RING_GO(64, 2, 4, 4) PDMK_RING_GO(128, 2, 3, 4) PDMK_RING_GO(64, 3, 4, 4)
        default: return 1;
    }
#undef PDMK_RING_GO
    return hipGetLastError() == hipSuccess ? 0 : -1000;
}

namespace pdmk_ring {
// ... 157 lines not shown
    if (do_colsum && (lane >> 4) == 0) {
#pragma unroll
        for (int i = 0; i < IMW; ++i) {
            const int m = m0 + wm * (16 * IMW) + i * 16 + (lane & 15);
            if (m < g.M) unsafeAtomicAdd(g.colsum_out + m, acs[i][0]);
        }
    }
    constexpr int SROW = 68;
    float* stage = reinterpret_cast<float*>(smem);
    const bool slab = g.accumulate == 2;
    float* Cf = reinterpret_cast<float*>(g.C) + (slab ? (long)wgc.by * g.M * g.ldc : 0L);
    const bool atomic = wgc.gy > 1 && !slab, acc1 = g.accumulate == 1;
#pragma unroll
    for (int t = 0; t < 9; ++t) {
        __syncthreads();
#pragma unroll
        for (int i = 0; i < IMW; ++i)
            *reinterpret_cast<f32x4*>(stage + (wm * (16 * IMW) + i * 16 + (lane & 15)) * SROW + wn * 16 + (lane >> 4) * 4) = acc[i][t];
        __syncthreads();
        const int ci = c0 + lane;
        if (ci < Ci) {
#pragma unroll
            for (int rr = 0; rr < BM / 8; ++rr) {
                const int row = wave * (BM / 8) + rr, m = m0 + row;
                if (m < g.M) {
                    const float v = stage[row * SROW + lane];
                    float* dst = Cf + (long)m * g.ldc + t * Ci + ci;
                    if (atomic) unsafeAtomicAdd(dst, v);
                    else *dst = acc1 ? *dst + v : v;
                }
            }
        }
    }
}

template <int IMW, int STAGES>
__global__ __launch_bounds__(NT, 1) void conv_wgrad_halo_kernel(pdmk_gemm_args g, unsigned a_bytes, unsigned b_bytes) {
    __shared__ __attribute__((aligned(1024))) unsigned char smem[wgrad_halo_smem_bytes(IMW, STAGES)];
    conv_wgrad_halo_body<IMW, STAGES>(g, a_bytes, b_bytes, PDMK_WGRAD_XCD ? lc_split_xcd() : lc_plain(), smem);
}
template <int IMW, int STAGES>
__global__ __launch_bounds__(NT, 1) void conv_wgrad_halo_group_kernel(pdmk_gemm_group_dev gg) {
    __shared__ __attribute__((aligned(1024))) unsigned char smem[wgrad_halo_smem_bytes(IMW, STAGES)];
    int pi;
    LC wgc;
    if (!lc_group(gg, pi, wgc)) return;
    conv_wgrad_halo_body<IMW, STAGES>(gg.p[pi], gg.a_bytes[pi], gg.b_bytes[pi], wgc, smem);
}

static bool wgrad_halo_ok(const pdmk_gemm_args& g) {
    if (g.dtype != PDMK_BF16 || g.a_mode != PDMK_A_COLK || g.b_mode != PDMK_B_COLK_CONV || !g.out_f32) return false;
    if (g.conv_mode != 0 || g.conv_ho != g.conv_hi || g.conv_wo != g.conv_wi || g.alpha != 1.0f) return false;
    if ((g.conv_ci % 8) || (g.conv_ld % 8) || (g.lda % 8) || (g.M % 8) || g.N != 9 * g.conv_ci || g.conv_wi < 4) return false;
    const int H = g.conv_hi, W = g.conv_wi, HW = H * W, W2 = (W + 2 + 7) & ~7;
    if (HW >= 128) return (HW % 128) == 0 && (128 % W) == 0 && (128 / W + 2) * W2 <= 288;
    return (128 % HW) == 0 && (128 / HW) * (H + 2) * W2 <= 288;
}

}

namespace {
struct GroupGrid {
    pdmk_gemm_group_dev gg;
    unsigned total = 0;
    void add(int i, const pdmk_gemm_args& g, int tiles, int splits, long ab, long bb, int aux0 = 0, int aux1 = 0) {
        gg.start[i] = (int)total;
        gg.gx[i] = tiles;
        gg.gy[i] = splits;
        gg.a_bytes[i] = (unsigned)ab;
        gg.b_bytes[i] = (unsigned)bb;
        gg.aux0[i] = aux0;
        gg.aux1[i] = aux1;
        gg.p[i] = g;
        total += ((unsigned)tiles * (unsigned)splits + 7u) & ~7u;
    }
    void finish(int n) {
        gg.n = n;
        for (int i = n; i <= PDMK_GEMM_GROUP_MAX; ++i) gg.start[i] = (int)total;
        for (int i = n; i < PDMK_GEMM_GROUP_MAX; ++i) {
            gg.gx[i] = gg.gy[i] = 0;
            gg.a_bytes[i] = gg.b_bytes[i] = 0;
            gg.aux0[i] = gg.aux1[i] = 0;
            gg.p[i] = gg.p[0];
        }
    }
};
}

int pdmk_gemm_ring_group_launch(const pdmk_gemm_args* gs, int n, hipStream_t st, const long* a_bytes, const long* b_bytes, int id) {
    using namespace pdmk_ring;
    if (n < 2 || n > PDMK_GEMM_GROUP_MAX || id < 0) return 1;
    const bool halo = id >= kNumBase && id < kNumBase + kNumHalo;
    if (id >= kNumConfigs + kNumHalo) return 1;
    const bool conv = gs[0].a_mode == PDMK_A_CONV;
    GroupGrid G;
    for (int i = 0; i < n; ++i) {
        const pdmk_gemm_args& g = gs[i];
        if (g.dtype != PDMK_BF16 || g.b_mode != PDMK_B_ROWK || g.a_mode == PDMK_A_COLK) return 1;
        if ((g.K % 8) || (g.a_mode == PDMK_A_CONV && (g.conv_ci % 8))) return 1;
        if ((g.a_mode == PDMK_A_CONV) != conv) return 1;
        if (!halo && g.a_mode == PDMK_A_CONV && g.conv_mode >= 5) return 1;
        const int sk = g.splitk > 1 ? g.splitk : 1;
        if (halo) {
            const int h = id - kNumBase;
            const int tw = halo_tile_w(g, h, g.splitk);
            if (tw <= 0) return 1;
            const int bm = h < 2 ? 256 : 128, bn = 32 * ((h & 1) ? 4 : 5);
            G.add(i, g, ((g.M + bm - 1) / bm) * ((g.N + bn - 1) / bn), sk, a_bytes[i], b_bytes[i], tw);
        } else {
            const Config c = kConfigs[id < kNumBase ? id : id - kNumHalo];
            const int bn = 32 * c.nj;
            G.add(i, g, ((g.M + c.bm - 1) / c.bm) * ((g.N + bn - 1) / bn), sk, a_bytes[i], b_bytes[i]);
        }
    }
    G.finish(n);
    const dim3 grid(G.total);
    if (halo) {
        bool phase = gs[0].conv_mode >= 5;
        for (int i = 1; i < n; ++i)
            if ((gs[i].conv_mode >= 5) != phase) return 1;
        if (phase) {
            if (id - kNumBase == 2) hipLaunchKernelGGL((conv_halo_group_kernel<128, 5, 4, 264, 4>), grid, dim3(NT), 0, st, G.gg);
            else hipLaunchKernelGGL((conv_halo_group_kernel<128, 4, 5, 264, 4>), grid, dim3(NT), 0, st, G.gg);
            return hipGetLastError() == hipSuccess ? 0 : -1000;
        }
        switch (id - kNumBase) {
            case 0: hipLaunchKernelGGL((conv_halo_group_kernel<256, 5, 3, 400>), grid, dim3(NT), 0, st, G.gg); break;
            case 1: hipLaunchKernelGGL((conv_halo_group_kernel<256, 4, 3, 400>), grid, dim3(NT), 0, st, G.gg); break;
            case 2: hipLaunchKernelGGL((conv_halo_group_kernel<128, 5, 4, 264>), grid, dim3(NT), 0, st, G.gg); break;
            default: hipLaunchKernelGGL((conv_halo_group_kernel<128, 4, 5, 264>), grid, dim3(NT), 0, st, G.gg); break;
        }
        return hipGetLastError() == hipSuccess ? 0 : -1000;
    }
    const Config c = kConfigs[id < kNumBase ? id : id - kNumHalo];
#define PDMK_RING_GGO(BMv, NJv, STv, OCv)                                                                             \
    case (BMv * 1000 + NJv * 100 + STv * 10 + OCv):                                                                   \
        if (conv) hipLaunchKernelGGL((igemm_ring_group_kernel<true, BMv, NJv, STv, OCv>), grid, dim3(NT), 0, st, G.gg); \
        else hipLaunchKernelGGL((igemm_ring_group_kernel<false, BMv, NJv, STv, OCv>), grid, dim3(NT), 0, st, G.gg);   \
        break;
    switch (c.bm * 1000 + c.nj * 100 + c.stages * 10 + c.occ) {
        PDMK_RING_GGO(256, 4, 3, 2) PDMK_RING_GGO(256, 5, 3, 2) PDMK_RING_GGO(128, 4, 4, 2) PDMK_RING_GGO(128, 5, 4, 2)
        PDMK_RING_GGO(64, 4, 6, 2) PDMK_RING_GGO(64, 5, 5, 2) PDMK_RING_GGO(128, 4, 2, 4) PDMK_RING_GGO(64, 4, 3, 4)
        PDMK_RING_GGO(64, 5, 2, 4) PDMK_RING_GGO(128, 6, 3, 2) PDMK_RING_GGO(64, 6, 4, 2) PDMK_RING_GGO(128, 5, 2, 4)
        PDMK_RING_GGO(64, 2, 4, 4) PDMK_RING_GGO(128, 2, 3, 4) PDMK_RING_GGO(64, 3, 4, 4)
        default: return 1;
    }
#undef PDMK_RING_GGO
    return hipGetLastError() == hipSuccess ? 0 : -1000;
}

struct WCfg { int bm, nj, stages, occ; };
static const WCfg kWCfgs[] = {{128, 4, 4, 2}, {128, 4, 2, 4}, {64, 4, 3, 4}, {128, 2, 3, 4}, {64, 2, 4, 4}};
constexpr int kNumW = sizeof(kWCfgs) / sizeof(kWCfgs[0]);
int pdmk_wgrad_ring_num_configs() { return kNumW + 2; }
int pdmk_wgrad_ring_name(int id, int conv, char* buf, int n) {
    if (id == kNumW || id == kNumW + 1) {
        snprintf(buf, n, "pdmk_ring::conv_wgrad_halo_kernel<%d, %d>", id == kNumW ? 2 : 4, id == kNumW ? 3 : 2);
        return 0;
    }
    if (id < 0 || id >= kNumW) return -1;
    const WCfg c = kWCfgs[id];
    snprintf(buf, n, "pdmk_ring::wgrad_ring_kernel<%s, %d, %d, %d, %d>", conv ? "true" : "false", c.bm, c.nj, c.stages, c.occ);
    return 0;
}
int pdmk_wgrad_ring_launch(const pdmk_gemm_args& g, hipStream_t st, long a_bytes, long b_bytes, int id) {
    using namespace pdmk_ring;
    if (g.dtype != PDMK_BF16 || g.a_mode != PDMK_A_COLK || g.b_mode == PDMK_B_ROWK || !g.out_f32) return 1;
    const bool conv = g.b_mode == PDMK_B_COLK_CONV;
    if ((g.M % 8) || (g.N % 8) || (g.lda % 8) || (!conv && (g.ldb % 8))) return 1;
    if (conv && ((g.conv_ci % 8) || (g.conv_ld % 8) || g.conv_mode == 3 || g.conv_mode == 4 || g.conv_mode > 8)) return 1;
    if (id == kNumW || id == kNumW + 1) {
        if (!wgrad_halo_ok(g)) return 1;
        const int nblk = (g.K + 127) / 128, sk = g.splitk > 1 ? g.splitk : 1, bm = id == kNumW ? 64 : 128;
        if (sk > nblk) return 1;
        dim3 grid(((g.M + bm - 1) / bm) * ((g.conv_ci + 63) / 64), sk);
        if (bm == 64) hipLaunchKernelGGL((conv_wgrad_halo_kernel<2, 3>), grid, dim3(NT), 0, st, g, (unsigned)a_bytes, (unsigned)b_bytes);
        else hipLaunchKernelGGL((conv_wgrad_halo_kernel<4, 2>), grid, dim3(NT), 0, st, g, (unsigned)a_bytes, (unsigned)b_bytes);
        return hipGetLastError() == hipSuccess ? 0 : -1000;
    }
    if (id < 0 || id >= kNumW) return 1;
    int lg_wo = -1, lg_howo = -1;
    if (conv) {
        auto lg = [](int v) { int l = 0; if (v <= 0 || (v & (v - 1))) return -1; while ((1 << l) < v) ++l; return l; };
        lg_wo = lg(g.conv_wo);
        lg_howo = lg(g.conv_ho * g.conv_wo);
        if (lg_wo < 0 || lg_howo < 0) lg_wo = lg_howo = -1;
    }
    const WCfg c = kWCfgs[id];
    const int bn = 32 * c.nj;
    dim3 grid(((g.M + c.bm - 1) / c.bm) * ((g.N + bn - 1) / bn), g.splitk > 1 ? g.splitk : 1);
#define PDMK_WG_GO(BMv, NJv, STv, OCv)                                                                                \
    case (BMv * 1000 + NJv * 100 + STv * 10 + OCv):                                                                   \
        if (conv) hipLaunchKernelGGL((wgrad_ring_kernel<true, BMv, NJv, STv, OCv>), grid, dim3(NT), 0, st, g, lg_wo,  \
                                     lg_howo, (unsigned)a_bytes, (unsigned)b_bytes);                                  \
        else hipLaunchKernelGGL((wgrad_ring_kernel<false, BMv, NJv, STv, OCv>), grid, dim3(NT), 0, st, g, lg_wo,      \
                                lg_howo, (unsigned)a_bytes, (unsigned)b_bytes);                                       \
        break;
    switch (c.bm * 1000 + c.nj * 100 + c.stages * 10 + c.occ) {
        PDMK_WG_GO(128, 4, 4, 2) PDMK_WG_GO(128, 4, 2, 4) PDMK_WG_GO(64, 4, 3, 4) PDMK_WG_GO(128, 2, 3, 4) PDMK_WG_GO(64, 2, 4, 4)
        default: return 1;
    }
#undef PDMK_WG_GO
    return hipGetLastError() == hipSuccess ? 0 : -1000;
}

int pdmk_wgrad_ring_group_launch(const pdmk_gemm_args* gs, int n, hipStream_t st, const long* a_bytes, const long* b_bytes, int id) {
    using namespace pdmk_ring;
    if (n < 2 || n > PDMK_GEMM_GROUP_MAX || id < 0 || id > kNumW + 1) return 1;
    const bool conv = gs[0].b_mode == PDMK_B_COLK_CONV;
    const bool halo = id == kNumW || id == kNumW + 1;
    GroupGrid G;
    for (int i = 0; i < n; ++i) {
        const pdmk_gemm_args& g = gs[i];
        if (g.dtype != PDMK_BF16 || g.a_mode != PDMK_A_COLK || g.b_mode == PDMK_B_ROWK || !g.out_f32) return 1;
        if ((g.b_mode == PDMK_B_COLK_CONV) != conv) return 1;
        if ((g.M % 8) || (g.N % 8) || (g.lda % 8) || (!conv && (g.ldb % 8))) return 1;
        if (conv && ((g.conv_ci % 8) || (g.conv_ld % 8) || g.conv_mode == 3 || g.conv_mode == 4 || g.conv_mode > 8)) return 1;
        const int sk = g.splitk > 1 ? g.splitk : 1;
        if (halo) {
            if (!wgrad_halo_ok(g)) return 1;
            const int nblk = (g.K + 127) / 128, bm = id == kNumW ? 64 : 128;
            if (sk > nblk) return 1;
            G.add(i, g, ((g.M + bm - 1) / bm) * ((g.conv_ci + 63) / 64), sk, a_bytes[i], b_bytes[i]);
        } else {
            int lg_wo = -1, lg_howo = -1;
            if (conv) {
                auto lg = [](int v) { int l = 0; if (v <= 0 || (v & (v - 1))) return -1; while ((1 << l) < v) ++l; return l; };
                lg_wo = lg(g.conv_wo);
                lg_howo = lg(g.conv_ho * g.conv_wo);
                if (lg_wo < 0 || lg_howo < 0) lg_wo = lg_howo = -1;
            }
            const WCfg c = kWCfgs[id];
            const int bn = 32 * c.nj;
            G.add(i, g, ((g.M + c.bm - 1) / c.bm) * ((g.N + bn - 1) / bn), sk, a_bytes[i], b_bytes[i], lg_wo, lg_howo);
        }
    }
    G.finish(n);
    const dim3 grid(G.total);
    if (halo) {
        if (id == kNumW) hipLaunchKernelGGL((conv_wgrad_halo_group_kernel<2, 3>), grid, dim3(NT), 0, st, G.gg);
        else hipLaunchKernelGGL((conv_wgrad_halo_group_kernel<4, 2>), grid, dim3(NT), 0, st, G.gg);
        return hipGetLastError() == hipSuccess ? 0 : -1000;
    }
    const WCfg c = kWCfgs[id];
#define PDMK_WG_GGO(BMv, NJv, STv, OCv)                                                                               \
    case (BMv * 1000 + NJv * 100 + STv * 10 + OCv):                                                                   \
        if (conv) hipLaunchKernelGGL((wgrad_ring_group_kernel<true, BMv, NJv, STv, OCv>), grid, dim3(NT), 0, st, G.gg); \
        else hipLaunchKernelGGL((wgrad_ring_group_kernel<false, BMv, NJv, STv, OCv>), grid, dim3(NT), 0, st, G.gg);   \
        break;
    switch (c.bm * 1000 + c.nj * 100 + c.stages * 10 + c.occ) {
        PDMK_WG_GGO(128, 4, 4, 2) PDMK_WG_GGO(128, 4, 2, 4) PDMK_WG_GGO(64, 4, 3, 4) PDMK_WG_GGO(128, 2, 3, 4) PDMK_WG_GGO(64, 2, 4, 4)
        default: return 1;
    }
#undef PDMK_WG_GGO
    return hipGetLastError() == hipSuccess ? 0 : -1000;
}
```

unlearn-ft_amd/pdm/_pdmk.py:

```python
import ctypes as C
import os

import torch

_HERE = os.path.dirname(os.path.abspath(__file__))
LIB_PATH = os.environ.get("PDMK_LIB") or os.path.join(os.path.dirname(_HERE), "libpdmk.so")

F32, BF16 = 0, 1
EPI_NONE, EPI_GEGLU, EPI_GEGLU_BWD = 0, 1, 2
A_ROWK, A_CONV, A_COLK = 0, 1, 2
B_ROWK, B_COLK, B_COLK_CONV = 0, 1, 2


class PdmkError(RuntimeError):
    pass


def _load():
    if not os.path.exists(LIB_PATH):
        raise PdmkError(f"libpdmk.so not found at {LIB_PATH}: build it with `python __graft_entry__.py` "
                        f"(or `make -C unlearn-ft_amd/csrc`); there is no CPU/PyTorch fallback for the hot path")
    return C.CDLL(LIB_PATH)


_lib = _load()

vp, i32, i64, f32, f64 = C.c_void_p, C.c_int32, C.c_int64, C.c_float, C.c_double


class GemmArgs(C.Structure):
    _fields_ = [("A", vp), ("B", vp), ("C", vp), ("bias", vp), ("rowvec", vp), ("R", vp), ("colsum_out", vp),
                ("M", i32), ("N", i32), ("K", i32),
                ("lda", i32), ("ldb", i32), ("ldc", i32), ("ldr", i32),
                ("rows_per_b", i32), ("a_mode", i32), ("b_mode", i32),
                ("conv_b", i32), ("conv_hi", i32), ("conv_wi", i32), ("conv_ci", i32), ("conv_ho", i32),
                ("conv_wo", i32), ("conv_mode", i32), ("conv_ld", i32),
                ("dtype", i32), ("out_f32", i32), ("accumulate", i32), ("splitk", i32), ("alpha", f32), ("ldrv", i32),
                ("epilogue", i32), ("ldc2", i32), ("C2", vp), ("colstat", vp), ("cs_ld", i32), ("cs_col0", i32),
                ("ln_gamma", vp), ("ln_beta", vp), ("ln_stats", vp), ("ln_out", vp), ("ld_ln_out", i32), ("ln_eps", f32)]


class PlmsRow(C.Structure):
    _fields_ = [("t", i64), ("mode", i32), ("nterms", i32), ("wslot", i32), ("rslot", i32 * 3), ("coef", f32 * 4),
                ("v_x", f32), ("v_v", f32), ("eps_scale", f32), ("x_scale", f32), ("vpred", i32), ("pad_", i32)]


_SIGS = {
    "pdmk_version": ([], i32),
    "pdmk_gemm": ([C.POINTER(GemmArgs), vp], i32),
    "pdmk_gemm_group": ([C.POINTER(GemmArgs), i32, vp, C.POINTER(i32)], i32),
    "pdmk_gemm_plan": ([C.POINTER(GemmArgs), vp, C.POINTER(i32)], i32),
    "pdmk_gemm_ln_supported": ([C.POINTER(GemmArgs)], i32),
    "pdmk_conv_up2_supported": ([i32, i32, i32, i32, i32, i32], i32),
    "pdmk_up2_pack_weights": ([vp, vp, vp, i32, i32, i32, vp], i32),
    "pdmk_up2_combine_wgrad": ([vp, vp, i32, i32, vp], i32),
    "pdmk_gemm_last_candidate": ([], i32),
    "pdmk_gemm_candidate_name": ([i32, i32, i32, C.c_char_p, i32], i32),
    "pdmk_splitk_finish": ([vp, vp, vp, vp, vp, i64, i32, i32, i32, i32, i32, i32, i32, i32, vp], i32),
    "pdmk_splitk_finish_colstat": ([vp, vp, vp, vp, vp, i64, i32, i32, i32, i32, i32, i32, i32, vp, i32, i32, i32, vp], i32),
    "pdmk_groupnorm_fwd": ([vp, vp, vp, vp, vp, vp, i32, i32, i32, i32, i32, i32, i32, f32, i32, i32, vp], i32),
    "pdmk_groupnorm_apply_colstat": ([vp, vp, vp, vp, vp, vp, i32, i32, i32, i32, i32, i32, i32, i32, i32, f32, i32, i32, vp], i32),
    "pdmk_groupnorm_bwd": ([vp, vp, vp, vp, vp, vp, vp, vp, vp, vp, i64, i32, i32, i32, i32, i32, i32, i32, i32, i32, i32, vp, i32, i32, vp], i32),
    "pdmk_groupnorm_bwd_partial_dims": ([i32, i32, i32, i32, i32, i32, C.POINTER(i32), C.POINTER(i32)], i32),
    "pdmk_layernorm_bwd_partial_dims": ([i32, i32, C.POINTER(i32), C.POINTER(i32)], i32),
    "pdmk_reduce_partials_group": ([vp, i32, vp], i32),
    "pdmk_splitk_finish_group": ([vp, i32, vp], i32),
    "pdmk_layernorm_fwd": ([vp, vp, vp, vp, vp, i32, i32, i32, i32, f32, i32, vp], i32),
    "pdmk_layernorm_bwd": ([vp, vp, vp, vp, vp, vp, vp, vp, i64, i32, i32, i32, i32, i32, i32, vp, i32, i32, vp], i32),
    "pdmk_attn_fwd": ([vp, vp, vp, vp, vp, i32, i32, i32, i32, i64, i32, i64, i32, i64, i32, i64, i32, f32, i32, vp], i32),
    "pdmk_attn_bwd": ([vp, vp, vp, vp, vp, vp, vp, vp, vp, vp, i32, i32, i32, i32,
                       i64, i32, i64, i32, i64, i32, i64, i32, i64, i32, i64, i32, i64, i32, f32, vp, i64, i32, vp], i32),
    "pdmk_geglu_fwd": ([vp, vp, i32, i32, i32, i32, i32, i32, vp], i32),
    "pdmk_geglu_bwd": ([vp, vp, vp, i32, i32, i32, i32, i32, i32, i32, vp], i32),
    "pdmk_quantize_e4m3": ([vp, vp, i64, i32, vp], i32),
    "pdmk_silu_fwd": ([vp, vp, i64, i32, vp], i32),
    "pdmk_silu_bwd": ([vp, vp, vp, i64, i32, vp], i32),
    "pdmk_copy2d": ([vp, vp, i64, i32, i32, i32, i32, i32, vp], i32),
    "pdmk_cast_permute": ([vp, vp, i32, i32, i32, i32, i32, vp], i32),
    "pdmk_colsum": ([vp, vp, i64, i32, i32, i32, i32, i32, i32, vp], i32),
    "pdmk_pool2x2_sum": ([vp, vp, i32, i32, i32, i32, i32, vp], i32),
    "pdmk_timestep_embed": ([vp, vp, vp, i32, i32, i32, vp], i32),
    "pdmk_add_noise_velocity": ([vp, vp, vp, vp, vp, vp, vp, i32, i32, i32, i32, i32, vp], i32),
    "pdmk_nchw_to_nhwc": ([vp, vp, i32, i32, i32, i32, i32, vp], i32),
    "pdmk_nhwc_to_nchw": ([vp, vp, i32, i32, i32, i32, i32, vp], i32),
    "pdmk_mse_fwd": ([vp, i32, vp, i32, vp, vp, i32, i32, i64, i32, i32, i32, f64, vp], i32),
    "pdmk_mse_bwd": ([vp, i32, vp, i32, vp, vp, i32, i64, i32, i32, i32, i32, f32, i32, vp], i32),
    "pdmk_mse_fwd_bwd": ([vp, i32, vp, i32, vp, vp, i32, vp, i32, i64, i32, i32, i32, i32, f64, f32, i32, vp], i32),
    "pdmk_axpby": ([vp, vp, f32, f32, i64, i32, vp], i32),
    "pdmk_adamw": ([vp, vp, vp, vp, i64, vp, f32, f32, f32, f32, vp, f32, i32, vp, vp], i32),
    "pdmk_transpose_tiles": ([vp, vp, vp, i32, i32, vp], i32),
    "pdmk_sumsq": ([vp, i64, vp, i32, vp], i32),
    "pdmk_zero": ([vp, i64, vp], i32),
    "pdmk_skinny_gemm": ([vp, i32, vp, vp, vp, i32, i32, i32, i32, i32, i32, i32, i32, i32, vp], i32),
    "pdmk_skinny_wgrad": ([vp, i32, vp, vp, vp, i32, i32, i32, i32, i32, i32, i32, vp], i32),
    "pdmk_softmax_rows": ([vp, vp, i64, i32, i64, i64, i32, vp], i32),
    "pdmk_latent_sample": ([vp, i32, vp, vp, i32, i32, i32, f32, i32, vp], i32),
    "pdmk_embed_tokens": ([vp, vp, vp, vp, i64, i32, i32, i32, i32, i32, i32, i32, vp], i32),
    "pdmk_attn_fwd_causal": ([vp, vp, vp, vp, vp, i32, i32, i32, i64, i32, i64, i32, i64, i32, i64, i32, f32, i32, vp], i32),
    "pdmk_gelu_fwd": ([vp, vp, i64, i32, vp], i32),
    "pdmk_image_prep": ([vp, i64, vp, vp, i32, i32, vp, vp], i32),
    "pdmk_image_prep_ex": ([vp, i64, vp, vp, i32, i32, i32, vp, vp, vp, vp], i32),
    "pdmk_patch_im2col": ([vp, vp, i32, i32, i32, i32, i32, vp], i32),
    "pdmk_vit_tokens": ([vp, i32, vp, vp, i32, vp, i32, i32, i32, i32, i32, vp], i32),
    "pdmk_quick_gelu_fwd": ([vp, vp, i64, i32, vp], i32),
    "pdmk_gather_rows": ([vp, i32, vp, i32, vp, i32, i32, i32, i32, vp], i32),
    "pdmk_clip_score_head": ([vp, i32, vp, i32, vp, vp, vp, i32, i32, vp], i32),
    "pdmk_plms_step": ([vp, i32, f32, f32, i32, vp, vp, vp, vp, i32, vp, vp, vp, i32, i32, i32, i32, i32, vp], i32),
    "pdmk_image_to_u8": ([vp, vp, i32, i32, i32, vp], i32),
    "pdmk_resize_bilinear_u8": ([vp, i64, vp, vp, i32, i32, vp, vp], i32),
    "pdmk_image_resize_u8": ([vp, i64, vp, vp, i32, i32, i32, vp, vp], i32),
    "pdmk_conv2d_fwd": ([vp, i32, vp, vp, vp, i32, i32, i32, i32, i32, i32, i32, i32, i32, i32, i32, i32, vp], i32),
    "pdmk_pool2d": ([vp, i32, vp, i32, i32, i32, i32, i32, i32, i32, i32, vp], i32),
    "pdmk_global_avgpool": ([vp, i32, vp, i32, i32, i32, vp], i32),
    "pdmk_fid_accumulate": ([vp, i32, i32, i32, vp, vp, vp], i32),
    "pdmk_gemm_splitk_workspace_bytes": ([i64, i32, i32], i64),
    "pdmk_groupnorm_workspace_bytes": ([i32, i32], i64),
    "pdmk_groupnorm_bwd_part_workspace_bytes": ([i32, i32], i64),
    "pdmk_layernorm_bwd_part_workspace_bytes": ([i32, i32], i64),
    "pdmk_attn_bwd_workspace_bytes": ([i32, i32, i32, i32], i64),
    "pdmk_plan_export": ([C.c_char_p], i32),
    "pdmk_plan_import": ([C.c_char_p], i32),
    "pdmk_plan_size": ([], i32),
    "pdmk_plan_clear": ([], i32),
    "pdmk_debug_scratch_violations": ([], i32),
    "pdmk_comm_unique_id": ([vp], i32),
    "pdmk_comm_create": ([vp, i32, i32, C.POINTER(vp)], i32),
    "pdmk_comm_allreduce_sum_f32": ([vp, vp, i64, vp], i32),
    "pdmk_comm_world": ([vp], i32),
    "pdmk_comm_rank": ([vp], i32),
    "pdmk_comm_reduce_scatter_sum_f32": ([vp, vp, i64, vp], i32),
    "pdmk_comm_allgather_f32": ([vp, vp, i64, vp], i32),
    "pdmk_stream_create": ([i32, C.POINTER(vp)], i32),
    "pdmk_stream_destroy": ([vp], i32),
    "pdmk_comm_destroy": ([vp], i32),
}
for _n, (_a, _r) in _SIGS.items():
    _f = getattr(_lib, _n)
    _f.argtypes, _f.restype = _a, _r

EXPORTS = tuple(_SIGS)


def version():
    return _lib.pdmk_version()


def dt(t):
    if t.dtype == torch.float32:
        return F32
    if t.dtype == torch.bfloat16:
        return BF16
    raise PdmkError(f"unsupported dtype {t.dtype}")


def _p(t):
    return None if t is None else t.data_ptr()


def _st():
    return torch.cuda.current_stream().cuda_stream


def _chk(rc, name):
    if rc != 0:
        raise PdmkError(f"{name} failed with status {rc}")


PROFILE = None

RECORD = None
TAG = ""
GROUP_MAX = 8
STATS = {"launches": 0, "grouped": 0}


class Rec:
    __slots__ = ("tag", "kind", "fn", "g", "keep", "macs", "meta")

    def __init__(self, kind, fn, g=None, keep=(), macs=None, meta=None):
        self.tag, self.kind, self.fn, self.g, self.keep, self.macs, self.meta = TAG, kind, fn, g, keep, macs, meta

    def run(self):
        self.fn()


class Recorder:

    def __enter__(self):
        global RECORD
        self.prev, self.recs = RECORD, []
        RECORD = self.recs
        return self

    def __exit__(self, *exc):
        global RECORD
        RECORD = self.prev
        return False


def _recordable(kind):
    def deco(fn):
        def wrapped(*a, **kw):
            if RECORD is not None:
                RECORD.append(Rec(kind, lambda: fn(*a, **kw)))
# ... 197 lines not shown
    key = (dev.index if dev.index is not None else torch.cuda.current_device(), role)
    s = _ROLE_STREAMS.get(key)
    if s is None:
        h = vp()
        with torch.cuda.device(key[0]):
            _chk(_lib.pdmk_stream_create(int(high_priority), C.byref(h)), "pdmk_stream_create")
        s = torch.cuda.ExternalStream(h.value, device=torch.device("cuda", key[0]))
        _ROLE_STREAMS[key] = s
    return s


def groupnorm_ws(device, B, G, have=None):
    need = _ws_bytes(_lib.pdmk_groupnorm_workspace_bytes(B, G)) // 8
    if have is not None and have.numel() >= need:
        return have
    return torch.empty(max(need, 1 << 17), device=device, dtype=torch.float64)


def zeros(shape, device, dtype):
    n = 1
    for d in shape:
        n *= d
    esz = torch.empty((), dtype=dtype).element_size()
    pad = (-(n * esz)) % 16 // esz
    flat = torch.empty(n + pad, device=device, dtype=dtype)
    _chk(_lib.pdmk_zero(_p(flat), (n + pad) * esz, _st()), "pdmk_zero")
    return flat[:n].view(*shape)


def zero_(t):
    assert t.is_contiguous() and (t.numel() * t.element_size()) % 16 == 0
    _chk(_lib.pdmk_zero(_p(t), t.numel() * t.element_size(), _st()), "pdmk_zero")
    return t


def last_candidate():
    return int(_lib.pdmk_gemm_last_candidate())


def candidate_name(a_mode, b_mode, cand):
    buf = C.create_string_buffer(160)
    _chk(_lib.pdmk_gemm_candidate_name(a_mode, b_mode, cand, buf, 160), "pdmk_gemm_candidate_name")
    return buf.value.decode()


def splitk_plan(A, B, M, N, K, lda, ldb, a_mode=A_ROWK, conv=None):
    g = GemmArgs()
    g.A, g.B = _p(A), _p(B)
    g.M, g.N, g.K = M, N, K
    g.lda, g.ldb, g.ldc = lda, ldb, N
    g.a_mode, g.b_mode = a_mode, B_ROWK
    if conv is not None:
        (g.conv_b, g.conv_hi, g.conv_wi, g.conv_ci, g.conv_ho, g.conv_wo, g.conv_mode, g.conv_ld) = conv
    g.dtype = dt(A)
    g.splitk, g.alpha = 1, 1.0
    sk = i32(1)
    _chk(_lib.pdmk_gemm_plan(C.byref(g), _st(), C.byref(sk)), "pdmk_gemm_plan")
    return int(sk.value)


def wgrad_plan(dy, x, M, N, K, lda, ldb, b_mode=B_COLK, conv=None, slabs=False):
    g = GemmArgs()
    g.accumulate = 2 if slabs else 0
    g.A, g.B = _p(dy), _p(x)
    g.M, g.N, g.K = M, N, K
    g.lda, g.ldb, g.ldc = lda, ldb, N
    g.a_mode, g.b_mode = A_COLK, b_mode
    if conv is not None:
        (g.conv_b, g.conv_hi, g.conv_wi, g.conv_ci, g.conv_ho, g.conv_wo, g.conv_mode, g.conv_ld) = conv
    g.dtype = dt(x)
    g.out_f32, g.splitk, g.alpha = 1, 1, 1.0
    sk = i32(1)
    _chk(_lib.pdmk_gemm_plan(C.byref(g), _st(), C.byref(sk)), "pdmk_gemm_plan")
    return int(sk.value)


def gemm_auto(A, B, Cout, M, N, K, lda, ldb, ldc, *, bias=None, rowvec=None, rows_per_b=0, R=None, ldr=0,
              a_mode=A_ROWK, conv=None, accumulate=False, macs=None, ldrv=0, colstat=None):
    sk = splitk_plan(A, B, M, N, K, lda, ldb, a_mode, conv)
    if sk == 1:
        gemm(A, B, Cout, M, N, K, lda, ldb, ldc, bias=bias, rowvec=rowvec, rows_per_b=rows_per_b, R=R, ldr=ldr,
             a_mode=a_mode, conv=conv, accumulate=accumulate, macs=macs, ldrv=ldrv, colstat=colstat)
        return colstat is not None
    ws = torch.empty(_ws_bytes(_lib.pdmk_gemm_splitk_workspace_bytes(M, N, sk)) // 4, device=A.device, dtype=torch.float32)
    gemm(A, B, ws, M, N, K, lda, ldb, N, a_mode=a_mode, conv=conv, out_f32=True, splitk=sk, accumulate=2, macs=macs)
    splitk_finish(ws, Cout, M, N, ldc, sk, bias=bias, rowvec=rowvec, R=R, ldr=ldr, rows_per_b=rows_per_b, ldrv=ldrv,
                  accumulate=accumulate, colstat=colstat)
    return colstat is not None


@_recordable("splitk_finish")
def splitk_finish(ws, Cout, M, N, ldc, nslab, *, bias=None, rowvec=None, R=None, ldr=0, rows_per_b=0, ldrv=0,
                  accumulate=False, colstat=None):
    if colstat is not None:
        _chk(_lib.pdmk_splitk_finish_colstat(_p(ws), _p(Cout), _p(bias), _p(rowvec), _p(R), M, N, ldc, ldr, rows_per_b, ldrv,
                                             nslab, int(accumulate), _p(colstat[0]), colstat[0].shape[2], int(colstat[1]),
                                             dt(Cout), _st()), "pdmk_splitk_finish_colstat")
        return
    _chk(_lib.pdmk_splitk_finish(_p(ws), _p(Cout), _p(bias), _p(rowvec), _p(R), M, N, ldc, ldr, rows_per_b, ldrv, nslab,
                                 int(accumulate), dt(Cout), _st()), "pdmk_splitk_finish")


class SlabItem(C.Structure):
    _fields_ = [("ws", vp), ("dst", vp), ("n", i64), ("nslab", i32), ("pad_", i32)]


SLAB_GROUP_MAX = 32


class SlabQueue:

    def __init__(self, max_bytes=1 << 30):
        self.items, self.bytes, self.max_bytes = [], 0, max_bytes

    def add(self, ws, dW, n, nslab):
        self.items.append((ws, dW, n, nslab))
        self.bytes += ws.numel() * 4

    def full(self):
        return len(self.items) >= SLAB_GROUP_MAX or self.bytes >= self.max_bytes

    def flush(self):
        while self.items:
            chunk, self.items = self.items[:SLAB_GROUP_MAX], self.items[SLAB_GROUP_MAX:]
            arr = (SlabItem * len(chunk))()
            for a, (ws, dW, n, nslab) in zip(arr, chunk):
                a.ws, a.dst, a.n, a.nslab = _p(ws), _p(dW), n, nslab
            _chk(_lib.pdmk_splitk_finish_group(C.cast(arr, vp), len(chunk), _st()), "pdmk_splitk_finish_group")
        self.bytes = 0


def wgrad(dy, x, dW, M, N, K, lda, ldb, *, b_mode=B_COLK, conv=None, colsum_out=None, macs=None, queue=None):
    if queue is not None and (M * N) % 4 == 0 and dW.is_contiguous():
        sk = wgrad_plan(dy, x, M, N, K, lda, ldb, b_mode, conv, slabs=True)
        if sk > 1:
            if queue.full():
                queue.flush()
            ws = torch.empty(sk * M * N, device=dy.device, dtype=torch.float32)
            gemm(dy, x, ws, M, N, K, lda, ldb, N, a_mode=A_COLK, b_mode=b_mode, conv=conv, out_f32=True, splitk=sk,
                 accumulate=2, dtype=dt(x), macs=macs, colsum_out=colsum_out)
            queue.add(ws, dW, M * N, sk)
            return
    else:
        sk = wgrad_plan(dy, x, M, N, K, lda, ldb, b_mode, conv)
    gemm(dy, x, dW, M, N, K, lda, ldb, N, a_mode=A_COLK, b_mode=b_mode, conv=conv, out_f32=True, splitk=sk,
         accumulate=(sk == 1), dtype=dt(x), macs=macs, colsum_out=colsum_out)


_WG_TARGET = int(os.environ.get("PDMK_WG_TARGET", "512"))
_WG_MINK = int(os.environ.get("PDMK_WG_MINK", "32"))
_WG_CONV_SLABS = os.environ.get("PDMK_WGRAD_SLABS_CONV", "0") == "1"


def wgrad_group(items, queue, target_wgs=None):
    items = [tuple(it) + (B_COLK, None) if len(it) == 10 else tuple(it) for it in items]
    while items:
        K, bm = items[0][5], items[0][10]
        same = [it for it in items if it[5] == K and it[10] == bm][:GROUP_MAX]
        items = [it for it in items if not any(it is s_ for s_ in same)]
        conv_g = bm == B_COLK_CONV
        tiles = sum(((it[3] + 127) // 128) * ((it[4] + 127) // 128) for it in same)
        nk = max(1, K // 64)
        sk = max(1, min((target_wgs or _WG_TARGET) // max(tiles, 1), nk // _WG_MINK, 64))
        if len(same) == 1 or (queue is None and not conv_g):
            for dy, x, dW, M, N, K_, lda, ldb, cs, macs, bm_, conv in same:
                wgrad(dy, x, dW, M, N, K_, lda, ldb, b_mode=bm_, conv=conv, colsum_out=cs, macs=macs, queue=None if conv_g else queue)
            continue
        with Recorder() as r:
            slabs = []
            for dy, x, dW, M, N, K_, lda, ldb, cs, macs, bm_, conv in same:
                if (not conv_g or _WG_CONV_SLABS) and queue is not None and sk > 1 and (M * N) % 4 == 0 and dW.is_contiguous():
                    ws = torch.empty(sk * M * N, device=dy.device, dtype=torch.float32)
                    gemm(dy, x, ws, M, N, K_, lda, ldb, N, a_mode=A_COLK, b_mode=bm_, conv=conv, out_f32=True, splitk=sk, accumulate=2,
                         dtype=dt(x), macs=macs, colsum_out=cs)
                    slabs.append((ws, dW, M * N, sk))
                else:
                    ska = sk if conv_g else 1
                    gemm(dy, x, dW, M, N, K_, lda, ldb, N, a_mode=A_COLK, b_mode=bm_, conv=conv, out_f32=True, splitk=ska,
                         accumulate=(ska == 1), dtype=dt(x), macs=macs, colsum_out=cs)
        gemm_group(r.recs)
        for ws, dW, n, nslab in slabs:
            if queue.full():
                queue.flush()
            queue.add(ws, dW, n, nslab)


@_recordable("groupnorm_apply_colstat")
def groupnorm_apply_colstat(x, y, gamma, beta, stats, colstat, col0, B, HW, Cc, ldx, ldy, G, gs, eps, silu):
    _chk(_lib.pdmk_groupnorm_apply_colstat(_p(x), _p(y), _p(gamma), _p(beta), _p(stats), _p(colstat), colstat.shape[2], int(col0),
                                           B, HW, Cc, ldx, ldy, G, gs, eps, int(silu), dt(x), _st()),
         "pdmk_groupnorm_apply_colstat")


@_recordable("groupnorm_fwd")
def groupnorm_fwd(x, y, gamma, beta, stats, ws, B, HW, Cc, ldx, ldy, G, gs, eps, silu):
    _chk(_lib.pdmk_groupnorm_fwd(_p(x), _p(y), _p(gamma), _p(beta), _p(stats), _p(ws), B, HW, Cc, ldx, ldy, G, gs,
                                 eps, int(silu), dt(x), _st()), "pdmk_groupnorm_fwd")


_PART_WS = {}


def part_ws(device, elems):
    buf = _PART_WS.get(device)
    if buf is None or buf.numel() < elems:
        buf = torch.empty(max(elems, 1 << 22), device=device, dtype=torch.float32)
        _PART_WS[device] = buf
    return buf


class PartialItem(C.Structure):
    _fields_ = [("part", vp), ("out0", vp), ("out1", vp), ("nblk", i32), ("n", i32)]


PARTIAL_GROUP_MAX = 32


class PartialQueue:

    def __init__(self):
        self.items = []

    def slab(self, device, nblk, n, dgamma, dbeta):
        if len(self.items) >= PARTIAL_GROUP_MAX:
            self.flush()
        t = torch.empty(nblk * 2 * n, device=device, dtype=torch.float32)
        self.items.append((t, dgamma, dbeta, nblk, n))
        return t

    def flush(self):
        while self.items:
            chunk, self.items = self.items[:PARTIAL_GROUP_MAX], self.items[PARTIAL_GROUP_MAX:]
            arr = (PartialItem * len(chunk))()
            for a, (t, g0, g1, nblk, n) in zip(arr, chunk):
                a.part, a.out0, a.out1, a.nblk, a.n = _p(t), _p(g0), _p(g1), nblk, n
            _chk(_lib.pdmk_reduce_partials_group(C.cast(arr, vp), len(chunk), _st()), "pdmk_reduce_partials_group")


def _dims(fn, *args):
    a, b = i32(0), i32(0)
    _chk(fn(*args, C.byref(a), C.byref(b)), fn.__name__)
    return a.value, b.value


def groupnorm_bwd(x, dy, dx, gamma, beta, stats, dgamma, dbeta, ws, B, HW, Cc, ldx, lddy, lddx, G, gs, silu, acc, add=None,
                  queue=None):
    if queue is not None:
        nblk, n = _dims(_lib.pdmk_groupnorm_bwd_partial_dims, B, HW, Cc, G, gs, dt(x))
        pw = queue.slab(x.device, nblk, n, dgamma, dbeta)
        dgamma = dbeta = None
    else:
        pw = part_ws(x.device, _ws_bytes(_lib.pdmk_groupnorm_bwd_part_workspace_bytes(G, gs)) // 4)
    _chk(_lib.pdmk_groupnorm_bwd(_p(x), _p(dy), _p(dx), _p(gamma), _p(beta), _p(stats), _p(dgamma), _p(dbeta), _p(ws),
                                 _p(pw), pw.numel(), B, HW, Cc, ldx, lddy, lddx, G, gs, int(silu), int(acc), _p(add),
                                 0 if add is None else add.stride(0), dt(x), _st()), "pdmk_groupnorm_bwd")


@_recordable("layernorm_fwd")
def layernorm_fwd(x, y, gamma, beta, stats, M, Cc, ldx, ldy, eps):
    _chk(_lib.pdmk_layernorm_fwd(_p(x), _p(y), _p(gamma), _p(beta), _p(stats), M, Cc, ldx, ldy, eps, dt(x), _st()),
         "pdmk_layernorm_fwd")


def layernorm_bwd(x, dy, dx, gamma, stats, dgamma, dbeta, M, Cc, ldx, lddy, lddx, acc, queue=None, add=None):
    if queue is not None:
        nblk, n = _dims(_lib.pdmk_layernorm_bwd_partial_dims, M, Cc)
        pw = queue.slab(x.device, nblk, n, dgamma, dbeta)
        dgamma = dbeta = None
    else:
        pw = part_ws(x.device, _ws_bytes(_lib.pdmk_layernorm_bwd_part_workspace_bytes(M, Cc)) // 4)
    _chk(_lib.pdmk_layernorm_bwd(_p(x), _p(dy), _p(dx), _p(gamma), _p(stats), _p(dgamma), _p(dbeta), _p(pw),
                                 pw.numel(), M, Cc, ldx, lddy, lddx, int(acc), _p(add), 0 if add is None else add.stride(0),
                                 dt(x), _st()), "pdmk_layernorm_bwd")


@_recordable("attn_fwd")
def attn_fwd(q, k, v, o, lse, B, H, Nq, Nk, qs, ks, vs, os_, scale):
    _chk(_lib.pdmk_attn_fwd(_p(q), _p(k), _p(v), _p(o), _p(lse), B, H, Nq, Nk, qs[0], qs[1], ks[0], ks[1], vs[0],
                            vs[1], os_[0], os_[1], scale, dt(q), _st()), "pdmk_attn_fwd")


def attn_bwd(q, k, v, o, do, lse, delta, dq, dk, dv, B, H, Nq, Nk, qs, ks, vs, os_, dqs, dks, dvs, scale):
    nws = _ws_bytes(_lib.pdmk_attn_bwd_workspace_bytes(B, H, Nq, Nk)) // 4
    ws = torch.empty(nws, device=q.device, dtype=torch.float32) if nws else None
    _chk(_lib.pdmk_attn_bwd(_p(q), _p(k), _p(v), _p(o), _p(do), _p(lse), _p(delta), _p(dq), _p(dk), _p(dv), B, H, Nq,
                            Nk, qs[0], qs[1], ks[0], ks[1], vs[0], vs[1], os_[0], os_[1], dqs[0], dqs[1], dks[0],
                            dks[1], dvs[0], dvs[1], scale, _p(ws), 0 if ws is None else ws.numel(), dt(q), _st()),
         "pdmk_attn_bwd")


@_recordable("geglu_fwd")
def geglu_fwd(x, y, M, Fd, ldx, ldy, layout=0):
    _chk(_lib.pdmk_geglu_fwd(_p(x), _p(y), M, Fd, ldx, ldy, int(layout), dt(x), _st()), "pdmk_geglu_fwd")


def geglu_bwd(x, dy, dx, M, Fd, ldx, lddy, lddx, layout=0):
    _chk(_lib.pdmk_geglu_bwd(_p(x), _p(dy), _p(dx), M, Fd, ldx, lddy, lddx, int(layout), dt(x), _st()), "pdmk_geglu_bwd")


_GEGLU_REFUSED = set()


def _launch_gemm_geglu(g, macs):
    if PROFILE is not None:
        e0, e1 = torch.cuda.Event(enable_timing=True), torch.cuda.Event(enable_timing=True)
        e0.record()
    rc = _lib.pdmk_gemm(C.byref(g), _st())
    if rc == -2:
        if not g.ln_gamma:
            _GEGLU_REFUSED.add((g.M, g.N, g.K))
        return False
    _chk(rc, "pdmk_gemm[geglu]")
    if PROFILE is not None:
        e1.record()
        PROFILE.append((("bf16", A_ROWK, B_ROWK, _lib.pdmk_gemm_last_candidate()), 2.0 * (macs if macs is not None else g.M * g.N * g.K),
                        e0, e1, (g.M, g.N, g.K, 1)))
    return True


def gemm_geglu(A, B, gl, f, M, N, K, lda, ldb, *, bias=None, macs=None, ln=None):
    if (M, N, K) in _GEGLU_REFUSED:
        return False
    g = GemmArgs()
    g.A, g.B, g.C, g.bias = _p(A), _p(B), _p(gl), _p(bias)
# ... 314 lines not shown
```

Measured before the change: 195.5 images/s.

## Add wide-tile wgrad kernels with autotuned grouped split-K plan

Adds new weight-gradient GEMM kernels with larger 160/320-wide tiles. They use a 5-stage LDS ring fed by buffer-load-to-LDS DMA and run as both single and grouped launches. A new group planner jointly tunes the kernel candidate and the split-K factor per wgrad group, pricing in the slab-reduction traffic. The per-GEMM split-K search bound now uses the minimum tile count across configs. Together these aim to raise MFMA utilisation and reuse in the backward weight GEMMs, at the cost of extra tuning time, more code paths and hand-written inline asm.

```diff
diff --git a/include/pdmk.h b/include/pdmk.h
--- a/include/pdmk.h
+++ b/include/pdmk.h
@@ -68,6 +68,9 @@
 #define PDMK_GEMM_GROUP_MAX 8
 int pdmk_gemm_group(const pdmk_gemm_args* args, int n, pdmk_stream stream, int32_t* grouped_out);
 int pdmk_gemm_plan(const pdmk_gemm_args* args, pdmk_stream stream, int32_t* splitk_out);
+int pdmk_wgrad_group_split(const pdmk_gemm_args* args, int n, int cand, int target_wgs, int min_ksteps);
+int pdmk_wgrad_group_plan(const pdmk_gemm_args* args, int n, int target_wgs, int min_ksteps, pdmk_stream stream,
+                          int32_t* cand_out, int32_t* splitk_out);
 int pdmk_gemm_last_candidate(void);
 int pdmk_gemm_candidate_name(int a_mode, int b_mode, int id, char* buf, int n);
 int pdmk_splitk_finish(const float* ws, void* C, const float* bias, const float* rowvec, const void* R, int64_t M,
diff --git a/unlearn-ft_amd/csrc/gemm.hip b/unlearn-ft_amd/csrc/gemm.hip
--- a/unlearn-ft_amd/csrc/gemm.hip
+++ b/unlearn-ft_amd/csrc/gemm.hip
@@ -452,6 +452,7 @@
 int pdmk_gemm_ring_pick(const pdmk_gemm_args& g);
 int pdmk_wgrad_ring_launch(const pdmk_gemm_args& g, hipStream_t st, long a_bytes, long b_bytes, int id);
 int pdmk_wgrad_ring_num_configs();
+int pdmk_wgrad_ring_tiles(int id, int M, int N, int conv_ci);
 
 static int env_int(const char* name, int def, int* cache) {
     static int dynamic = -1;
@@ -860,6 +861,7 @@
 namespace {
 
 std::map<std::vector<int>, int> g_group_plan;
+std::map<std::vector<int>, std::pair<int, int>> g_wgroup_plan;
 
 int member_plan(const pdmk_gemm_args& g, hipStream_t st) {
     const int sk = g.splitk > 1 ? g.splitk : 1;
@@ -941,13 +943,13 @@
     }, st, e0, e1);
     int best = -1;
     float bt = t_sep * 0.98f;
-    int cands[PDMK_GEMM_GROUP_MAX + 12], nc = 0;
+    int cands[PDMK_GEMM_GROUP_MAX + 24], nc = 0;
     for (int i = 0; i < n; ++i) cands[nc++] = ids[i];
     cands[nc++] = heuristic_cfg(a[0]);
     if (a[0].a_mode == PDMK_A_CONV)
         for (int h = 0; h < 4; ++h) cands[nc++] = 1 + 12 + h;
     if (a[0].a_mode == PDMK_A_COLK && a[0].b_mode == PDMK_B_COLK)
-        for (int w = 0; w < 5; ++w) cands[nc++] = 1 + w;
+        for (int w = 0; w < pdmk_wgrad_ring_num_configs(); ++w) cands[nc++] = 1 + w;
     for (int i = 0; i < nc; ++i) {
         bool seen = cands[i] <= 0;
         for (int j = 0; j < i; ++j) seen = seen || cands[j] == cands[i];
@@ -1039,6 +1041,166 @@
     return separate();
 }
 
+namespace {
+
+int wgrad_tiles(const pdmk_gemm_args& g, int cand) {
+    if (cand <= 0) return ((g.M + 127) / 128) * ((g.N + 127) / 128);
+    return pdmk_wgrad_ring_tiles(cand - 1, g.M, g.N, g.b_mode == PDMK_B_COLK_CONV ? g.conv_ci : 0);
+}
+
+int wgrad_group_split(const pdmk_gemm_args* a, int n, int cand, int target_wgs, int min_ksteps) {
+    long tiles = 0;
+    for (int i = 0; i < n; ++i) tiles += wgrad_tiles(a[i], cand);
+    const long nk = a[0].K / 64 > 0 ? a[0].K / 64 : 1;
+    if (tiles < 1) tiles = 1;
+    long s = (target_wgs + tiles - 1) / tiles;
+    if (s > nk / min_ksteps) s = nk / min_ksteps;
+    if (s > 64) s = 64;
+    return s < 1 ? 1 : (int)s;
+}
+
+void wgroup_args(const pdmk_gemm_args* a, int n, int sk, pdmk_gemm_args* out) {
+    for (int i = 0; i < n; ++i) {
+        out[i] = a[i];
+        out[i].splitk = sk;
+        out[i].accumulate = sk == 1 ? 1 : (a[i].accumulate == 2 ? 2 : 0);
+    }
+}
+
+std::vector<int> group_key(const pdmk_gemm_args* a, int n) {
+    std::vector<int> key;
+    for (int i = 0; i < n; ++i) {
+        const PlanKey k = make_key(a[i], a[i].splitk > 1 ? a[i].splitk : 1);
+        key.insert(key.end(), k.v, k.v + 10);
+        key.push_back(a[i].accumulate);
+    }
+    return key;
+}
+
+std::pair<int, int> tune_wgroup(const pdmk_gemm_args* a, int n, int target_wgs, int min_ksteps, hipStream_t st) {
+    const int ncand = 1 + pdmk_wgrad_ring_num_configs();
+    const int sk0 = wgrad_group_split(a, n, 0, target_wgs, min_ksteps);
+    const std::pair<int, int> none(-1, sk0);
+    int sk_of[64], sk_max = sk0;
+    for (int c = 1; c < ncand && c < 64; ++c) {
+        sk_of[c] = wgrad_group_split(a, n, c, target_wgs, min_ksteps);
+        sk_max = std::max(sk_max, sk_of[c]);
+    }
+    size_t off[PDMK_GEMM_GROUP_MAX + 1];
+    off[0] = 0;
+    for (int i = 0; i < n; ++i) {
+        const size_t out = (size_t)a[i].M * (size_t)a[i].N * 4;
+        off[i + 1] = off[i] + ((out * (size_t)sk_max + (size_t)a[i].M * 4 + 1023) & ~(size_t)1023);
+    }
+    {
+        std::lock_guard<std::mutex> lk(g_plan_mu);
+        if (!ensure_scratch(off[n] + 256)) return none;
+    }
+    pdmk_gemm_args t[PDMK_GEMM_GROUP_MAX];
+    auto prep = [&](int sk) -> float {
+        wgroup_args(a, n, sk, t);
+        float sum_us = 0.f;
+        for (int i = 0; i < n; ++i) {
+            char* base = reinterpret_cast<char*>(g_scratch) + off[i];
+            t[i].C = base;
+            t[i].ldc = a[i].N;
+            if (t[i].accumulate == 1) t[i].accumulate = 0;
+            if (t[i].colsum_out)
+                t[i].colsum_out = reinterpret_cast<float*>(base + (off[i + 1] - off[i]) - (((size_t)a[i].M * 4 + 15) & ~(size_t)15));
+            if (t[i].accumulate == 2) sum_us += (float)(sk + 1) * (float)a[i].M * (float)a[i].N * 4.f / 4.0e6f;
+        }
+        return sum_us;
+    };
+    pdmk_gemm_args f[PDMK_GEMM_GROUP_MAX];
+    int ids[PDMK_GEMM_GROUP_MAX];
+    wgroup_args(a, n, sk0, f);
+    for (int i = 0; i < n; ++i) ids[i] = member_plan(f[i], st);
+    (void)hipDeviceSynchronize();
+    hipEvent_t e0, e1;
+    if (hipEventCreate(&e0) != hipSuccess || hipEventCreate(&e1) != hipSuccess) { (void)hipGetLastError(); return none; }
+    float price = prep(sk0);
+    const float t_sep = price + time_us([&]() -> int {
+        for (int i = 0; i < n; ++i) {
+            int rc = launch_candidate(t[i], st, ids[i]);
+            if (rc == 1) rc = launch_legacy(t[i], st);
+            if (rc) return rc;
+        }
+        return 0;
+    }, st, e0, e1);
+    std::pair<int, int> best = none;
+    float bt = t_sep * 0.98f;
+    for (int c = 1; c < ncand && c < 64; ++c)
+        for (int pass = 0; pass < 2; ++pass) {
+            const int sk = pass ? sk0 : sk_of[c];
+            if (pass && (sk == sk_of[c] || c > 7)) continue;
+            price = prep(sk);
+            const float tg = price + time_us([&]() -> int { return group_launch(t, n, st, c); }, st, e0, e1);
+            if (getenv("PDMK_TUNE_LOG") && tg < 1e29f) fprintf(stderr, "[pdmk wgroup]   cand %d sk %d: %.1f us\n", c, sk, tg);
+            if (tg < bt) { bt = tg; best = std::make_pair(c, sk); }
+        }
+    (void)hipEventDestroy(e0);
+    (void)hipEventDestroy(e1);
+    if (getenv("PDMK_TUNE_LOG")) {
+        fprintf(stderr, "[pdmk wgroup] n=%d", n);
+        for (int i = 0; i < n; ++i) fprintf(stderr, " (%d,%d,%d)", a[i].M, a[i].N, a[i].K);
+        fprintf(stderr, " separate sk %d %.1f us -> cand %d sk %d (%.1f us)\n", sk0, t_sep, best.first, best.second, best.first > 0 ? bt : t_sep);
+    }
+    {
+        std::lock_guard<std::mutex> lk(g_plan_mu);
+        if (!scratch_check()) return none;
+    }
+    return best;
+}
+
+}
+
+extern "C" int pdmk_wgrad_group_split(const pdmk_gemm_args* a, int n, int cand, int target_wgs, int min_ksteps) {
+    if (!a || n < 1 || n > PDMK_GEMM_GROUP_MAX || cand < 0 || cand > pdmk_wgrad_ring_num_configs() || target_wgs < 1 || min_ksteps < 1)
+        return -1;
+    for (int i = 0; i < n; ++i)
+        if (a[i].M <= 0 || a[i].N <= 0 || a[i].K <= 0 || a[i].K != a[0].K) return -1;
+    return wgrad_group_split(a, n, cand, target_wgs, min_ksteps);
+}
+
+extern "C" int pdmk_wgrad_group_plan(const pdmk_gemm_args* a, int n, int target_wgs, int min_ksteps, pdmk_stream stream,
+                                     int32_t* cand_out, int32_t* splitk_out) {
+    if (!cand_out || !splitk_out) return -1;
+    const int sk0 = pdmk_wgrad_group_split(a, n, 0, target_wgs, min_ksteps);
+    if (sk0 < 1) return -1;
+    *cand_out = 0;
+    *splitk_out = sk0;
+    hipStream_t st = reinterpret_cast<hipStream_t>(stream);
+    bool wg = n > 1;
+    for (int i = 0; i < n; ++i) wg = wg && wgrad_eligible(a[i]) && a[i].b_mode == a[0].b_mode && a[i].A && a[i].B && !(a[i].N & 3);
+    if (!wg || !group_mode() || !ring_mode() || forced_cfg() >= 0 || forced_wcfg() >= 0 || forced_group() >= 1) return 0;
+    std::vector<int> key;
+    for (int i = 0; i < n; ++i) {
+        const PlanKey k = make_key(a[i], 0);
+        key.insert(key.end(), k.v, k.v + 10);
+    }
+    key.push_back(target_wgs);
+    key.push_back(min_ksteps);
+    {
+        std::lock_guard<std::mutex> lk(g_plan_mu);
+        auto it = g_wgroup_plan.find(key);
+        if (it != g_wgroup_plan.end()) {
+            *cand_out = it->second.first;
+            *splitk_out = it->second.second;
+            return 0;
+        }
+    }
+    if (!can_tune(st)) return 0;
+    const std::pair<int, int> best = tune_wgroup(a, n, target_wgs, min_ksteps, st);
+    pdmk_gemm_args f[PDMK_GEMM_GROUP_MAX];
+    wgroup_args(a, n, best.second, f);
+    std::lock_guard<std::mutex> lk(g_plan_mu);
+    g_wgroup_plan[key] = best;
+    g_group_plan[group_key(f, n)] = best.first;
+    *cand_out = best.first;
+    *splitk_out = best.second;
+    return 0;
+}
+
 extern "C" int pdmk_gemm_last_candidate(void) { return g_last_candidate; }
 int pdmk_gemm_ring_name(int id, int conv, char* buf, int n);
 int pdmk_wgrad_ring_name(int id, int conv, char* buf, int n);
@@ -1075,6 +1237,12 @@
     if (it != g_plan_sk.end()) { *splitk_out = it->second; return 0; }
     if (!can_tune(st) || !a->A || !a->B) { *splitk_out = wg ? heuristic_wgrad_sk(g) : heuristic_sk(g); return 0; }
     const int tiles = ((g.M + 127) / 128) * ((g.N + 127) / 128);
+    int tiles_min = tiles;
+    if (wg)
+        for (int id = 0; id < pdmk_wgrad_ring_num_configs(); ++id) {
+            const int t = pdmk_wgrad_ring_tiles(id, g.M, g.N, 0);
+            if (t > 0 && t < tiles_min) tiles_min = t;
+        }
     const int nk = (g.K + 63) / 64;
     const int cands[12] = {1, 2, 3, 4, 6, 8, 12, 16, 24, 32, 48, 64};
     int best_sk = 1;
@@ -1082,7 +1250,7 @@
     for (int c = 0; c < 12; ++c) {
         const int sk = cands[c];
         if (wg) {
-            if (sk > 1 && (nk / sk < 4 || (long)tiles * sk > 1280)) continue;
+            if (sk > 1 && (nk / sk < 4 || (long)tiles_min * sk > 1280)) continue;
             if ((long)tiles * sk * 4 < 128 && sk < 64 && nk / (2 * sk) >= 4) continue;
         } else if (sk > 16 || (sk > 1 && (tiles > 200 || nk < 10 || nk / sk < 3 || (long)tiles * sk > 768))) continue;
         float t = 1e30f;
@@ -1144,6 +1312,7 @@
     g_plan_cfg.clear();
     g_plan_sk.clear();
     g_group_plan.clear();
+    g_wgroup_plan.clear();
     if (g_scratch) (void)hipFree(g_scratch);
     g_scratch = nullptr;
     g_scratch_bytes = 0;
@@ -1155,4 +1324,4 @@
     return g_scratch_violations;
 }
 
-extern "C" int pdmk_version(void) { return 121; }
+extern "C" int pdmk_version(void) { return 122; }
diff --git a/unlearn-ft_amd/csrc/gemm_ring.hip b/unlearn-ft_amd/csrc/gemm_ring.hip
--- a/unlearn-ft_amd/csrc/gemm_ring.hip
+++ b/unlearn-ft_amd/csrc/gemm_ring.hip
@@ -2,6 +2,8 @@
 
 #include <stdio.h>
 #include <stdlib.h>
+
+#include <type_traits>
 
 #ifndef PDMK_WGRAD_XCD
 #define PDMK_WGRAD_XCD 1
@@ -964,6 +966,255 @@
     wgrad_ring_body<CONV, BM, NJ, STAGES, OCC>(gg.p[pi], gg.aux0[pi], gg.aux1[pi], gg.a_bytes[pi], gg.b_bytes[pi], wgc, smem);
 }
 
+constexpr int WBK = 32, WSTAGES = 5, WF = 5;
+typedef int i32x4 __attribute__((ext_vector_type(4)));
+__device__ __forceinline__ i32x4 dma_rsrc(const void* p, unsigned bytes) {
+    const unsigned long a = (unsigned long)p;
+    i32x4 r;
+    r[0] = __builtin_amdgcn_readfirstlane((int)(unsigned)a);
+    r[1] = __builtin_amdgcn_readfirstlane((int)((unsigned)(a >> 32) & 0xffffu));
+    r[2] = __builtin_amdgcn_readfirstlane((int)bytes);
+    r[3] = 0x00020000;
+    return r;
+}
+__device__ __forceinline__ void dma16_hidden(i32x4 rsrc, unsigned lds_addr, unsigned voff) {
+    unsigned keep;
+    asm volatile("s_nop 4\n\ts_mov_b32 %0, m0\n\ts_mov_b32 m0, %2\n\ts_nop 0\n\tbuffer_load_dwordx4 %1, %3, 0 offen lds\n\ts_mov_b32 m0, %0"
+                 : "=&s"(keep) : "v"(voff), "s"(lds_addr), "s"(rsrc) : "memory");
+}
+constexpr int wide_smem_bytes(int BM, int BN) { return WSTAGES * WBK * (BM + BN) * 2; }
+__device__ __forceinline__ int wide_swz(int rbytes, int k) {
+    return rbytes == 640 ? (((k >> 1) & 1) | (((k >> 3) & 1) << 1)) : ((k >> 3) & 1);
+}
+
+template <bool CONV, int WM, int WN>
+__device__ __forceinline__ void wgrad_wide_body(const pdmk_gemm_args& g, int lg_wo, int lg_howo, unsigned a_bytes, unsigned b_bytes,
+                                                const LC wgc, unsigned char* smem) {
+    typedef Mma<bf16> MM;
+    constexpr int BM = 16 * WF * WM, BN = 16 * WF * WN;
+    constexpr int RA = BM * 2, RB = BN * 2;
+    constexpr int A_BYTES = WBK * RA, SLOT = WBK * (RA + RB);
+    constexpr int PA = A_BYTES / 1024, NP = SLOT / 1024, PW = (NP + 7) / 8;
+    static_assert(WM * WN == 8 && (RA == 320 || RA == 640) && (RB == 320 || RB == 640), "tile");
+    static_assert(A_BYTES % 1024 == 0 && SLOT % 1024 == 0 && WSTAGES * SLOT <= 160 * 1024, "ring must fit the 160 KiB LDS");
+    static_assert(WSTAGES * SLOT == wide_smem_bytes(BM, BN), "smem size of the kernel wrappers");
+
+    const int tid = threadIdx.x, lane = tid & 63, wave = __builtin_amdgcn_readfirstlane(tid >> 6);
+    const int wm = wave / WN, wn = wave % WN;
+    const int ntn = (g.N + BN - 1) / BN;
+    const int tile = xcd_remap(wgc.bx, wgc.gx);
+    const int m0 = (tile / ntn) * BM, n0 = (tile % ntn) * BN;
+    const int nk_total = (g.K + WBK - 1) / WBK;
+    const int per64 = ((g.K + 63) / 64 + wgc.gy - 1) / wgc.gy;
+    const int kt0 = wgc.by * per64 * 2;
+    const int kt1 = min(nk_total, kt0 + per64 * 2);
+    if (kt0 >= kt1 && g.accumulate != 2) return;
+
+    const i32x4 rsrcA = dma_rsrc(g.A, a_bytes), rsrcB = dma_rsrc(g.B, b_bytes);
+    const unsigned lds0 = __builtin_amdgcn_readfirstlane((unsigned)(unsigned long)(__attribute__((address_space(3))) unsigned char*)smem);
+    const ConvGeom cg{g.conv_hi, g.conv_wi, g.conv_ci, g.conv_ho, g.conv_wo, g.conv_ld, g.conv_mode};
+
+    const int npw = (NP - wave + 7) / 8;
+    int p_k[PW], p_c[PW], p_ci[CONV ? PW : 1];
+#pragma unroll
+    for (int i = 0; i < PW; ++i) {
+        const int piece = i * 8 + wave;
+        const bool isA = piece < PA;
+        const int cpr = (isA ? RA : RB) / 16;
+        const int pos = (isA ? piece : piece - PA) * 64 + lane;
+        const int k = pos / cpr, cp = pos - k * cpr;
+        const int col = (isA ? m0 : n0) + ((cp ^ (wide_swz(isA ? RA : RB, k) << 1)) << 3);
+        const bool ok = col < (isA ? g.M : g.N);
+        p_k[i] = k;
+        p_c[i] = ok ? col : -1;
+        if (CONV) {
+            p_ci[i] = 0;
+            if (!isA) {
+                const int tap = col / cg.ci;
+                p_ci[i] = col - tap * cg.ci;
+                p_c[i] = ok ? tap : -1;
+            }
+        }
+    }
+
+    auto issue = [&](int kt, int slot) {
+        const unsigned s = lds0 + (unsigned)(slot * SLOT);
+#pragma unroll
+        for (int i = 0; i < PW; ++i) {
+            const int piece = i * 8 + wave;
+            if (piece >= NP) break;
+            const int kr = kt * WBK + p_k[i];
+            unsigned v = OOB;
+            if (piece < PA) {
+                unsigned krs = (unsigned)kr;
+                if (CONV && cg.mode >= 5 && kr < g.K) {
+                    const int hw = cg.ho * cg.wo, b = kr / hw, rem = kr - b * hw, oy = rem / cg.wo, ox = rem - oy * cg.wo;
+                    const int ph = cg.mode - 5;
+                    krs = (unsigned)((b * 2 * cg.ho + 2 * oy + (ph >> 1)) * (2 * cg.wo) + 2 * ox + (ph & 1));
+                }
+                if (kr < g.K && p_c[i] >= 0) v = (krs * (unsigned)g.lda + (unsigned)p_c[i]) * 2u;
+                dma16_hidden(rsrcA, s + (unsigned)(piece * 1024), v);
+            } else {
+                if (CONV) {
+                    if (kr < g.K && p_c[i] >= 0) {
+                        int b, oy, ox;
+                        if (lg_wo >= 0) {
+                            b = kr >> lg_howo;
+                            const int rem = kr & ((1 << lg_howo) - 1);
+                            oy = rem >> lg_wo;
+                            ox = rem & ((1 << lg_wo) - 1);
+                        } else {
+                            const int hw = cg.ho * cg.wo;
+                            b = kr / hw;
+                            const int rem = kr - b * hw;
+                            oy = rem / cg.wo;
+                            ox = rem - oy * cg.wo;
+                        }
+                        const int px = conv_src_pixel(cg, b, oy, ox, p_c[i]);
+                        if (px >= 0) v = ((unsigned)px * (unsigned)cg.ld + (unsigned)p_ci[i]) * 2u;
+                    }
+                } else if (kr < g.K && p_c[i] >= 0) {
+                    v = ((unsigned)kr * (unsigned)g.ldb + (unsigned)p_c[i]) * 2u;
+                }
+                dma16_hidden(rsrcB, s + (unsigned)(piece * 1024), v);
+            }
+        }
+    };
+
+    const int nfm = max(0, min(WF, (g.M - m0 - wm * (16 * WF)) >> 4)), nfn = max(0, min(WF, (g.N - n0 - wn * (16 * WF)) >> 4));
+
+    f32x4 acc[WF][WF], acs = f32x4{0.f, 0.f, 0.f, 0.f};
+#pragma unroll
+    for (int i = 0; i < WF; ++i)
+#pragma unroll
+        for (int j = 0; j < WF; ++j) acc[i][j] = f32x4{0.f, 0.f, 0.f, 0.f};
+    const bool do_colsum = g.colsum_out != nullptr && n0 == 0 && wn == 0;
+    const unsigned short one_bits = 0x3f80;
+
+    const int tg = lane >> 4, tq = (lane & 15) >> 2, tp = lane & 3, tk = 8 * tg + tq;
+    unsigned aoff[WF], boff[WF];
+#pragma unroll
+    for (int i = 0; i < WF; ++i) {
+        const int ca = (wm * (16 * WF) + i * 16) >> 3, cb = (wn * (16 * WF) + i * 16) >> 3;
+        aoff[i] = (unsigned)(tk * RA + ((ca ^ (wide_swz(RA, tk) << 1)) | (tp >> 1)) * 16 + (tp & 1) * 8);
+        boff[i] = (unsigned)(A_BYTES + tk * RB + ((cb ^ (wide_swz(RB, tk) << 1)) | (tp >> 1)) * 16 + (tp & 1) * 8);
+    }
+    typedef __attribute__((address_space(3))) s16x4 lds_s16x4;
+    auto tr_frag = [&](const unsigned char* a0, int rbytes) -> bf16x8 {
+        s16x4 lo = __builtin_amdgcn_ds_read_tr16_b64_v4i16((lds_s16x4*)(a0));
+        s16x4 hi = __builtin_amdgcn_ds_read_tr16_b64_v4i16((lds_s16x4*)(a0 + 4 * rbytes));
+        s16x8 v = __builtin_shufflevector(lo, hi, 0, 1, 2, 3, 4, 5, 6, 7);
+        return __builtin_bit_cast(bf16x8, v);
+    };
+
+#pragma unroll
+    for (int s = 0; s < WSTAGES - 1; ++s)
+        if (kt0 + s < kt1) issue(kt0 + s, s);
+
+    auto kloop = [&](auto nfm_c, auto nfn_c) {
+        constexpr int NFM = decltype(nfm_c)::value, NFN = decltype(nfn_c)::value;
+        int slot = 0;
+        for (int kt = kt0; kt < kt1; ++kt) {
+            wait_vmcnt_dyn(min(WSTAGES - 2, kt1 - 1 - kt) * npw);
+            __builtin_amdgcn_s_barrier();
+            if (kt + WSTAGES - 1 < kt1) issue(kt + WSTAGES - 1, slot == 0 ? WSTAGES - 1 : slot - 1);
+            __builtin_amdgcn_sched_barrier(0);
+            const unsigned char* ss = smem + slot * SLOT;
+            if (NFM > 0 && NFN > 0) {
+                bf16x8 af[NFM > 0 ? NFM : 1], bf[NFN > 0 ? NFN : 1];
+#pragma unroll
+                for (int i = 0; i < NFM; ++i) af[i] = tr_frag(ss + aoff[i], RA);
+#pragma unroll
+                for (int j = 0; j < NFN; ++j) bf[j] = tr_frag(ss + boff[j], RB);
+#pragma unroll
+                for (int i = 0; i < NFM; ++i)
+#pragma unroll
+                    for (int j = 0; j < NFN; ++j) acc[i][j] = MM::mma(bf[j], af[i], acc[i][j]);
+                if (do_colsum) {
+#pragma unroll
+                    for (int i = 0; i < NFM; ++i) {
+                        s16x8 sel;
+#pragma unroll
+                        for (int e = 0; e < 8; ++e) sel[e] = (short)((lane & 15) == i ? one_bits : 0);
+                        acs = MM::mma(__builtin_bit_cast(bf16x8, sel), af[i], acs);
+                    }
+                }
+            }
+            slot = slot + 1 == WSTAGES ? 0 : slot + 1;
+        }
+    };
+    using std::integral_constant;
+    typedef integral_constant<int, WF> FullC;
+    if (nfm == 0 || nfn == 0) kloop(integral_constant<int, 0>{}, integral_constant<int, 0>{});
+    else if (nfn == WF) {
+        switch (nfm) {
+            case 1: kloop(integral_constant<int, 1>{}, FullC{}); break;
+            case 2: kloop(integral_constant<int, 2>{}, FullC{}); break;
+            case 3: kloop(integral_constant<int, 3>{}, FullC{}); break;
+            case 4: kloop(integral_constant<int, 4>{}, FullC{}); break;
+            default: kloop(FullC{}, FullC{}); break;
+        }
+    } else if (nfm == WF) {
+        switch (nfn) {
+            case 1: kloop(FullC{}, integral_constant<int, 1>{}); break;
+            case 2: kloop(FullC{}, integral_constant<int, 2>{}); break;
+            case 3: kloop(FullC{}, integral_constant<int, 3>{}); break;
+            default: kloop(FullC{}, integral_constant<int, 4>{}); break;
+        }
+    } else kloop(FullC{}, FullC{});
+    if (do_colsum) {
+#pragma unroll
+        for (int i = 0; i < WF; ++i) {
+            const int m = m0 + wm * (16 * WF) + i * 16 + (lane & 15);
+            if (i < nfm && (lane >> 4) == (i >> 2)) unsafeAtomicAdd(g.colsum_out + m, acs[i & 3]);
+        }
+    }
+    const bool slab = g.accumulate == 2;
+    const bool atomic = wgc.gy > 1 && !slab;
+    const bool acc1 = g.accumulate == 1;
+    float* Cf = reinterpret_cast<float*>(g.C) + (slab ? (long)wgc.by * g.M * g.ldc : 0L);
+#pragma unroll
+    for (int i = 0; i < WF; ++i) {
+        if (i >= nfm) break;
+        const int m = m0 + wm * (16 * WF) + i * 16 + (lane & 15);
+#pragma unroll
+        for (int j = 0; j < WF; ++j) {
+            if (j >= nfn) continue;
+            const int n = n0 + wn * (16 * WF) + j * 16 + (lane >> 4) * 4;
+            f32x4 v = acc[i][j];
+#pragma unroll
+            for (int r = 0; r < 4; ++r) v[r] *= g.alpha;
+            float* dst = Cf + (long)m * g.ldc + n;
+            if (atomic) {
+#pragma unroll
+                for (int r = 0; r < 4; ++r) unsafeAtomicAdd(dst + r, v[r]);
+            } else {
+                if (acc1) {
+                    const f32x4 c = *reinterpret_cast<const f32x4*>(dst);
+#pragma unroll
+                    for (int r = 0; r < 4; ++r) v[r] += c[r];
+                }
+                *reinterpret_cast<f32x4*>(dst) = v;
+            }
+        }
+        __builtin_amdgcn_sched_barrier(0);
+    }
+}
+
+template <bool CONV, int WM, int WN>
+__global__ __launch_bounds__(NT, 1) void wgrad_wide_kernel(pdmk_gemm_args g, int lg_wo, int lg_howo, unsigned a_bytes, unsigned b_bytes) {
+    __shared__ __attribute__((aligned(1024))) unsigned char smem[wide_smem_bytes(80 * WM, 80 * WN)];
+    wgrad_wide_body<CONV, WM, WN>(g, lg_wo, lg_howo, a_bytes, b_bytes, PDMK_WGRAD_XCD ? lc_split_xcd() : lc_plain(), smem);
+}
+template <bool CONV, int WM, int WN>
+__global__ __launch_bounds__(NT, 1) void wgrad_wide_group_kernel(pdmk_gemm_group_dev gg) {
+    __shared__ __attribute__((aligned(1024))) unsigned char smem[wide_smem_bytes(80 * WM, 80 * WN)];
+    int pi;
+    LC wgc;
+    if (!lc_group(gg, pi, wgc)) return;
+    wgrad_wide_body<CONV, WM, WN>(gg.p[pi], gg.aux0[pi], gg.aux1[pi], gg.a_bytes[pi], gg.b_bytes[pi], wgc, smem);
+}
+
 struct Config {
     int bm, nj, stages, occ;
 };
@@ -1427,8 +1678,31 @@
 struct WCfg { int bm, nj, stages, occ; };
 static const WCfg kWCfgs[] = {{128, 4, 4, 2}, {128, 4, 2, 4}, {64, 4, 3, 4}, {128, 2, 3, 4}, {64, 2, 4, 4}};
 constexpr int kNumW = sizeof(kWCfgs) / sizeof(kWCfgs[0]);
-int pdmk_wgrad_ring_num_configs() { return kNumW + 2; }
+constexpr int kWide0 = kNumW + 2, kNumWAll = kNumW + 4;
+int pdmk_wgrad_ring_num_configs() { return kNumWAll; }
+int pdmk_wgrad_ring_tiles(int id, int M, int N, int conv_ci) {
+    if (id < 0 || id >= kNumWAll) return 0;
+    if (id == kNumW || id == kNumW + 1) return ((M + (id == kNumW ? 63 : 127)) / (id == kNumW ? 64 : 128)) * ((conv_ci + 63) / 64);
+    const int bm = id == kWide0 ? 320 : id == kWide0 + 1 ? 160 : kWCfgs[id].bm;
+    const int bn = id == kWide0 ? 160 : id == kWide0 + 1 ? 320 : 32 * kWCfgs[id].nj;
+    return ((M + bm - 1) / bm) * ((N + bn - 1) / bn);
+}
+static bool wgrad_wide_ok(const pdmk_gemm_args& g) {
+    return (g.M % 16) == 0 && (g.N % 16) == 0 && (g.ldc % 4) == 0 && (((uintptr_t)g.C) & 15) == 0 && !g.bias && !g.rowvec && !g.R;
+}
+static void wgrad_lg(const pdmk_gemm_args& g, bool conv, int* lg_wo, int* lg_howo) {
+    *lg_wo = *lg_howo = -1;
+    if (!conv) return;
+    auto lg = [](int v) { int l = 0; if (v <= 0 || (v & (v - 1))) return -1; while ((1 << l) < v) ++l; return l; };
+    *lg_wo = lg(g.conv_wo);
+    *lg_howo = lg(g.conv_ho * g.conv_wo);
+    if (*lg_wo < 0 || *lg_howo < 0) *lg_wo = *lg_howo = -1;
+}
 int pdmk_wgrad_ring_name(int id, int conv, char* buf, int n) {
+    if (id == kWide0 || id == kWide0 + 1) {
+        snprintf(buf, n, "pdmk_ring::wgrad_wide_kernel<%s, %d, %d>", conv ? "true" : "false", id == kWide0 ? 4 : 2, id == kWide0 ? 2 : 4);
+        return 0;
+    }
     if (id == kNumW || id == kNumW + 1) {
         snprintf(buf, n, "pdmk_ring::conv_wgrad_halo_kernel<%d, %d>", id == kNumW ? 2 : 4, id == kNumW ? 3 : 2);
         return 0;
@@ -1453,13 +1727,18 @@
         else hipLaunchKernelGGL((conv_wgrad_halo_kernel<4, 2>), grid, dim3(NT), 0, st, g, (unsigned)a_bytes, (unsigned)b_bytes);
         return hipGetLastError() == hipSuccess ? 0 : -1000;
     }
-    if (id < 0 || id >= kNumW) return 1;
-    int lg_wo = -1, lg_howo = -1;
-    if (conv) {
-        auto lg = [](int v) { int l = 0; if (v <= 0 || (v & (v - 1))) return -1; while ((1 << l) < v) ++l; return l; };
-        lg_wo = lg(g.conv_wo);
-        lg_howo = lg(g.conv_ho * g.conv_wo);
-        if (lg_wo < 0 || lg_howo < 0) lg_wo = lg_howo = -1;
+    if (id < 0 || id >= kNumWAll) return 1;
+    int lg_wo, lg_howo;
+    wgrad_lg(g, conv, &lg_wo, &lg_howo);
+    if (id >= kWide0) {
+        if (!wgrad_wide_ok(g)) return 1;
+        dim3 grid(pdmk_wgrad_ring_tiles(id, g.M, g.N, 0), g.splitk > 1 ? g.splitk : 1);
+#define PDMK_WW_GO(CV, WMv, WNv)                                                                                      \
+    hipLaunchKernelGGL((wgrad_wide_kernel<CV, WMv, WNv>), grid, dim3(NT), 0, st, g, lg_wo, lg_howo, (unsigned)a_bytes, (unsigned)b_bytes)
+        if (id == kWide0) { if (conv) PDMK_WW_GO(true, 4, 2); else PDMK_WW_GO(false, 4, 2); }
+        else { if (conv) PDMK_WW_GO(true, 2, 4); else PDMK_WW_GO(false, 2, 4); }
+#undef PDMK_WW_GO
+        return hipGetLastError() == hipSuccess ? 0 : -1000;
     }
     const WCfg c = kWCfgs[id];
     const int bn = 32 * c.nj;
@@ -1481,7 +1760,7 @@
 
 int pdmk_wgrad_ring_group_launch(const pdmk_gemm_args* gs, int n, hipStream_t st, const long* a_bytes, const long* b_bytes, int id) {
     using namespace pdmk_ring;
-    if (n < 2 || n > PDMK_GEMM_GROUP_MAX || id < 0 || id > kNumW + 1) return 1;
+    if (n < 2 || n > PDMK_GEMM_GROUP_MAX || id < 0 || id >= kNumWAll) return 1;
     const bool conv = gs[0].b_mode == PDMK_B_COLK_CONV;
     const bool halo = id == kNumW || id == kNumW + 1;
     GroupGrid G;
@@ -1498,16 +1777,10 @@
             if (sk > nblk) return 1;
             G.add(i, g, ((g.M + bm - 1) / bm) * ((g.conv_ci + 63) / 64), sk, a_bytes[i], b_bytes[i]);
         } else {
-            int lg_wo = -1, lg_howo = -1;
-            if (conv) {
-                auto lg = [](int v) { int l = 0; if (v <= 0 || (v & (v - 1))) return -1; while ((1 << l) < v) ++l; return l; };
-                lg_wo = lg(g.conv_wo);
-                lg_howo = lg(g.conv_ho * g.conv_wo);
-                if (lg_wo < 0 || lg_howo < 0) lg_wo = lg_howo = -1;
-            }
-            const WCfg c = kWCfgs[id];
-            const int bn = 32 * c.nj;
-            G.add(i, g, ((g.M + c.bm - 1) / c.bm) * ((g.N + bn - 1) / bn), sk, a_bytes[i], b_bytes[i], lg_wo, lg_howo);
+            int lg_wo, lg_howo;
+            wgrad_lg(g, conv, &lg_wo, &lg_howo);
+            if (id >= kWide0 && !wgrad_wide_ok(g)) return 1;
+            G.add(i, g, pdmk_wgrad_ring_tiles(id, g.M, g.N, 0), sk, a_bytes[i], b_bytes[i], lg_wo, lg_howo);
         }
     }
     G.finish(n);
@@ -1515,6 +1788,16 @@
     if (halo) {
         if (id == kNumW) hipLaunchKernelGGL((conv_wgrad_halo_group_kernel<2, 3>), grid, dim3(NT), 0, st, G.gg);
         else hipLaunchKernelGGL((conv_wgrad_halo_group_kernel<4, 2>), grid, dim3(NT), 0, st, G.gg);
+        return hipGetLastError() == hipSuccess ? 0 : -1000;
+    }
+    if (id >= kWide0) {
+        if (id == kWide0) {
+            if (conv) hipLaunchKernelGGL((wgrad_wide_group_kernel<true, 4, 2>), grid, dim3(NT), 0, st, G.gg);
+            else hipLaunchKernelGGL((wgrad_wide_group_kernel<false, 4, 2>), grid, dim3(NT), 0, st, G.gg);
+        } else {
+            if (conv) hipLaunchKernelGGL((wgrad_wide_group_kernel<true, 2, 4>), grid, dim3(NT), 0, st, G.gg);
+            else hipLaunchKernelGGL((wgrad_wide_group_kernel<false, 2, 4>), grid, dim3(NT), 0, st, G.gg);
+        }
         return hipGetLastError() == hipSuccess ? 0 : -1000;
     }
     const WCfg c = kWCfgs[id];
diff --git a/unlearn-ft_amd/pdm/_pdmk.py b/unlearn-ft_amd/pdm/_pdmk.py
--- a/unlearn-ft_amd/pdm/_pdmk.py
+++ b/unlearn-ft_amd/pdm/_pdmk.py
@@ -50,6 +50,8 @@
     "pdmk_gemm": ([C.POINTER(GemmArgs), vp], i32),
     "pdmk_gemm_group": ([C.POINTER(GemmArgs), i32, vp, C.POINTER(i32)], i32),
     "pdmk_gemm_plan": ([C.POINTER(GemmArgs), vp, C.POINTER(i32)], i32),
+    "pdmk_wgrad_group_split": ([C.POINTER(GemmArgs), i32, i32, i32, i32], i32),
+    "pdmk_wgrad_group_plan": ([C.POINTER(GemmArgs), i32, i32, i32, vp, C.POINTER(i32), C.POINTER(i32)], i32),
     "pdmk_gemm_ln_supported": ([C.POINTER(GemmArgs)], i32),
     "pdmk_conv_up2_supported": ([i32, i32, i32, i32, i32, i32], i32),
     "pdmk_up2_pack_weights": ([vp, vp, vp, i32, i32, i32, vp], i32),
@@ -553,6 +555,28 @@
 _WG_CONV_SLABS = os.environ.get("PDMK_WGRAD_SLABS_CONV", "0") == "1"
 
 
+def _wgrad_group_args(same, slab_ok):
+    arr = (GemmArgs * len(same))()
+    for g, (dy, x, dW, M, N, K_, lda, ldb, cs, macs, bm_, conv), ok in zip(arr, same, slab_ok):
+        g.A, g.B, g.C, g.colsum_out = _p(dy), _p(x), _p(dW), _p(cs)
+        g.M, g.N, g.K, g.lda, g.ldb, g.ldc = M, N, K_, lda, ldb, N
+        g.a_mode, g.b_mode = A_COLK, bm_
+        if conv is not None:
+            (g.conv_b, g.conv_hi, g.conv_wi, g.conv_ci, g.conv_ho, g.conv_wo, g.conv_mode, g.conv_ld) = conv
+        g.dtype, g.out_f32, g.splitk, g.alpha, g.accumulate = dt(x), 1, 1, 1.0, (2 if ok else 0)
+    return arr
+
+
+def wgrad_group_split(shapes, K, cand=0, target_wgs=None, min_ksteps=None):
+    arr = (GemmArgs * len(shapes))()
+    for g, (M, N) in zip(arr, shapes):
+        g.M, g.N, g.K, g.a_mode, g.b_mode = M, N, K, A_COLK, B_COLK
+    sk = _lib.pdmk_wgrad_group_split(arr, len(shapes), cand, target_wgs or _WG_TARGET, min_ksteps or _WG_MINK)
+    if sk < 1:
+        raise PdmkError("pdmk_wgrad_group_split rejected its arguments")
+    return int(sk)
+
+
 def wgrad_group(items, queue, target_wgs=None):
     items = [tuple(it) + (B_COLK, None) if len(it) == 10 else tuple(it) for it in items]
     while items:
@@ -560,17 +584,20 @@
         same = [it for it in items if it[5] == K and it[10] == bm][:GROUP_MAX]
         items = [it for it in items if not any(it is s_ for s_ in same)]
         conv_g = bm == B_COLK_CONV
-        tiles = sum(((it[3] + 127) // 128) * ((it[4] + 127) // 128) for it in same)
-        nk = max(1, K // 64)
-        sk = max(1, min((target_wgs or _WG_TARGET) // max(tiles, 1), nk // _WG_MINK, 64))
         if len(same) == 1 or (queue is None and not conv_g):
             for dy, x, dW, M, N, K_, lda, ldb, cs, macs, bm_, conv in same:
                 wgrad(dy, x, dW, M, N, K_, lda, ldb, b_mode=bm_, conv=conv, colsum_out=cs, macs=macs, queue=None if conv_g else queue)
             continue
+        slab_ok = [(not conv_g or _WG_CONV_SLABS) and queue is not None and (it[3] * it[4]) % 4 == 0 and it[2].is_contiguous()
+                   for it in same]
+        cand, sk = i32(0), i32(1)
+        _chk(_lib.pdmk_wgrad_group_plan(_wgrad_group_args(same, slab_ok), len(same), target_wgs or _WG_TARGET, _WG_MINK, _st(),
+                                        C.byref(cand), C.byref(sk)), "pdmk_wgrad_group_plan")
+        sk = int(sk.value)
         with Recorder() as r:
             slabs = []
-            for dy, x, dW, M, N, K_, lda, ldb, cs, macs, bm_, conv in same:
-                if (not conv_g or _WG_CONV_SLABS) and queue is not None and sk > 1 and (M * N) % 4 == 0 and dW.is_contiguous():
+            for (dy, x, dW, M, N, K_, lda, ldb, cs, macs, bm_, conv), ok in zip(same, slab_ok):
+                if ok and sk > 1:
                     ws = torch.empty(sk * M * N, device=dy.device, dtype=torch.float32)
                     gemm(dy, x, ws, M, N, K_, lda, ldb, N, a_mode=A_COLK, b_mode=bm_, conv=conv, out_f32=True, splitk=sk, accumulate=2,
                          dtype=dt(x), macs=macs, colsum_out=cs)
```

Result: no change. 197.0 images/s, median of 6 (+0.8%).
